# ahtamjidi/3PRE

Hardware: AMD Instinct MI355X
Metric: EKF steps/sec (predict+RANSAC+update) at N=500 landmarks; P-update %MFMA peak (higher is better)
Workload: dtype f32

## Files before the change

### 3pre_amd/csrc/pre3_api.hip

```cpp
#include <time.h>
#include <algorithm>
#include <immintrin.h>
#include <cmath>
#include <cstdarg>
#include <new>

#include <chrono>
#include "pre3_internal.h"
#include "pre3_test_hooks.h"
#include "pre3_geomdev.h"
#include <mutex>
#include "pre3_cholp.h"

namespace pre3 {

static thread_local char g_err[512] = "";
void set_error(const char *fmt, ...)
{
    va_list ap; va_start(ap, fmt);
    vsnprintf(g_err, sizeof g_err, fmt, ap);
    va_end(ap);
}

template <typename T> static int dmalloc(T **p, size_t count)
// ... 142 lines not shown
            if (t0 == 0) t0 = t;
            else if (t - t0 > 2.0) break;
        }
    }
    PRE3_TRY(stream_drain(c, __func__));
    if (__atomic_load_n(w, __ATOMIC_ACQUIRE) != seq) {
        c->stage_seq[k] = 0;
        (void)hipMemsetAsync(c->chol_arrive + 8 + k, 0, sizeof(unsigned int), c->stream);
        set_error("staging block %d: its pull has not run", k);
        return PRE3_E_STATE;
    }
    return PRE3_OK;
}
static StageDone stage_done(pre3_ctx *c, int k) { return StageDone{ c->chol_arrive + 8 + k, c->mail_dev + 16 + k, ++c->stage_seq[k] }; }

int launch_pull(pre3_ctx *c, const void *pinned_host, void *dst_dev, size_t bytes, int done_slot)
{
    void *src_dev = nullptr;
    PRE3_HIP(hipHostGetDevicePointer(&src_dev, const_cast<void *>(pinned_host), 0));
    const int n16 = (int)((bytes + 15) / 16);
    if (n16 == 0) return PRE3_OK;
    hipLaunchKernelGGL(k_scan_pull, dim3(ceil_div(n16, 256)), dim3(256), 0, c->stream, (const int4 *)src_dev, n16, (int4 *)dst_dev, 0, (int4 *)nullptr,
                       done_slot >= 0 ? stage_done(c, done_slot) : StageDone{ nullptr, nullptr, 0 });
    PRE3_HIP(hipGetLastError());
    return PRE3_OK;
}

int install_measurements(pre3_ctx *c, int m, const int32_t *meas_idx, const double *z, const int32_t *hyp, int n_hyp_ints, bool flags_clear, bool pull, size_t *nbytes_out)
{
    PRE3_CHECK(m >= 0 && m <= c->capm, PRE3_E_ARG, "measurements: m=%d exceeds capacity %d", m, c->capm);
    for (int j = 0; j < m; ++j) {
        PRE3_CHECK(meas_idx[j] >= 0 && meas_idx[j] < c->N, PRE3_E_ARG, "measurements: landmark index %d out of range", meas_idx[j]);
        PRE3_CHECK(j == 0 || meas_idx[j] > meas_idx[j - 1], PRE3_E_ARG, "measurements: landmark indices must be strictly ascending");
    }
    if (c->inbox_pending) { PRE3_TRY(wait_mail(c, 10, c->seq_inbox)); c->inbox_pending = false; }
    c->m = m; c->meas_host.assign(meas_idx, meas_idx + m);
    c->carry.select_pending = false;
    int32_t *hm = (int32_t *)(c->inbox_host + c->off_meas), *hic = (int32_t *)(c->inbox_host + c->off_ic);
    double *hz = (double *)(c->inbox_host + c->off_z);
    memset(hic, 0, sizeof(int32_t) * c->N);
    for (int j = 0; j < m; ++j) { hm[j] = meas_idx[j]; hic[meas_idx[j]] = 1; }
    if (z) {
        memset(hz, 0, sizeof(double) * 2 * c->N);
        for (int j = 0; j < m; ++j) { hz[2 * meas_idx[j]] = z[2 * j]; hz[2 * meas_idx[j] + 1] = z[2 * j + 1]; }
    }
    if (hyp) memcpy(c->inbox_host + c->off_hyp, hyp, sizeof(int32_t) * n_hyp_ints);
    const size_t nbytes = z ? c->off_z + sizeof(double) * 2 * c->N : c->off_hyp + (hyp ? sizeof(int32_t) * n_hyp_ints : 0);
    int32_t *const flags = (int32_t *)((unsigned char *)c->inbox_dev + c->off_flags);
    if (pull) { PRE3_TRY(launch_inbox_pull(c, c->inbox_host_dev, c->inbox_dev, (nbytes + 15) / 16, ++c->seq_inbox, 10, flags_clear ? nullptr : flags, flags_clear ? 0 : (int)(c->flags_bytes / 4))); c->inbox_pending = true; }
    if (nbytes_out) *nbytes_out = nbytes;
    if (!flags_clear && !pull) PRE3_HIP(hipMemsetAsync(flags, 0, c->flags_bytes, c->stream));
    c->li_from_host = c->hi_from_host = -1; c->li_kernel = c->hi_kernel = false;
    c->hp_all_valid = false;
    c->measurements_set = true;
    return PRE3_OK;
}

}

using namespace pre3;

extern "C" {

const char *pre3_last_error(void) { return pre3::g_err; }
const char *pre3_version(void) { return "pre3-mi355x 0.1 (gfx950)"; }

int pre3_device_count(void)
{
    int n = 0;
    if (hipGetDeviceCount(&n) != hipSuccess) return 0;
    return n;
}

static int pend_alloc(pre3_ctx *c)
{
    if (c->W_pend && c->Wp_pend && c->hf_xy) return PRE3_OK;
    PRE3_CHECK(c->dtype == PRE3_F32 && c->Wp != nullptr && c->rcap >= 2 * NB, PRE3_E_STATE, "PRE3_OPT_PEND_HI: fp32 contexts with the persistent factorisation only");
    int rc = PRE3_OK;
    auto A = [&](int r) { if (rc == PRE3_OK) rc = r; };
    if (!c->W_pend) { void *f = nullptr; A(dmalloc_bytes(&f, (size_t)2 * NB * c->ldw * sizeof(float))); c->W_pend = (float *)f; }
    if (!c->Wp_pend) A(dmalloc_bytes(&c->Wp_pend, (size_t)ceil_div(c->ldw, 128) * (c->rcap / 16) * (3 * 4 * 64) * 16));
    if (!c->hf_xy) { void *f = nullptr; A(dmalloc_bytes(&f, sizeof(unsigned) * 256)); c->hf_xy = (unsigned *)f; }
    return rc;
}

static int tail_alloc(pre3_ctx *c)
{
    if (c->tail_yp && c->tail_hb && c->tail_hib && c->tail_wt) return PRE3_OK;
    PRE3_CHECK(c->dtype == PRE3_F32 && c->Wp != nullptr, PRE3_E_STATE, "PRE3_OPT_STEP_TAIL: fp32 contexts with the persistent factorisation only");
    int rc = PRE3_OK;
    auto A = [&](int r) { if (rc == PRE3_OK) rc = r; };
    if (!c->tail_yp) A(dmalloc_bytes(&c->tail_yp, (size_t)(c->capN + 1) * 2 * 3 * c->rcap * 2));
    if (!c->tail_hb) { void *f = nullptr; A(dmalloc_bytes(&f, (size_t)c->capN * 2 * 16 * sizeof(float))); c->tail_hb = (float *)f; }
    if (!c->tail_hib) { void *f = nullptr; A(dmalloc_bytes(&f, sizeof(int32_t) * (64 + 64 * 16))); c->tail_hib = (int32_t *)f; }
    if (!c->tail_wt) { void *f = nullptr; A(dmalloc_bytes(&f, (size_t)c->ldw * c->rcap * sizeof(float))); c->tail_wt = (float *)f; }
    return rc;
}

int pre3_create(pre3_ctx **out, int device, int dtype, int max_landmarks, int max_hyp)
{
    PRE3_CHECK(out != nullptr, PRE3_E_ARG, "pre3_create: null output pointer");
    *out = nullptr;
    PRE3_CHECK(dtype == PRE3_F64 || dtype == PRE3_F32, PRE3_E_ARG, "pre3_create: dtype must be PRE3_F64 or PRE3_F32");
    PRE3_CHECK(max_landmarks >= 1 && max_hyp >= 1, PRE3_E_ARG, "pre3_create: capacities must be >= 1");
    int ndev = 0;
    if (hipGetDeviceCount(&ndev) != hipSuccess || ndev <= 0) { set_error("no HIP device available (libpre3 has no CPU fallback)"); return PRE3_E_NODEVICE; }
    PRE3_CHECK(device >= 0 && device < ndev, PRE3_E_NODEVICE, "pre3_create: device %d out of range (have %d)", device, ndev);
    PRE3_HIP(hipSetDevice(device));
    pre3_ctx *c = new (std::nothrow) pre3_ctx();
    PRE3_CHECK(c != nullptr, PRE3_E_NOMEM, "out of host memory");
    c->device = device; c->dtype = dtype; c->esz = dtype == PRE3_F64 ? 8 : 4;
    c->capN = max_landmarks; c->capn = 13 + 6 * max_landmarks; c->capm = max_landmarks; c->caph = max_hyp;
    c->ld = round_up(c->capn, TILE); c->ldw = c->ld + NB;
    { const char *e = getenv("PRE3_TAIL"); c->step_tail = e ? atoi(e) != 0 : false; }
    c->rcap = round_up(2 * c->capm, NB) + NB;
    c->mask_words_cap = ceil_div(c->capm, 32);
    int rc = PRE3_OK;
    auto A = [&](int r) { if (rc == PRE3_OK) rc = r; };
    if (hipStreamCreateWithFlags(&c->stream, hipStreamNonBlocking) != hipSuccess) { set_error("hipStreamCreate failed"); delete c; return PRE3_E_HIP; }
    A(dmalloc(&c->x_kk, c->capn)); A(dmalloc(&c->x_km1, c->capn));
    A(dmalloc_bytes(&c->P, (size_t)c->ld * c->ld * c->esz));
    A(dmalloc(&c->lm.type, c->capN)); A(dmalloc(&c->lm.off, c->capN));
    A(dmalloc(&c->lm.h, 2 * (size_t)c->capN)); A(dmalloc(&c->lm.has_h, c->capN));
    A(dmalloc(&c->lm.Hc, 14 * (size_t)c->capN)); A(dmalloc(&c->lm.Hl, 12 * (size_t)c->capN));
    A(dmalloc(&c->lm.S, 4 * (size_t)c->capN)); A(dmalloc(&c->lm.has_S, c->capN));
    {
        c->off_meas = 0;
        c->off_ic = c->off_meas + sizeof(int32_t) * c->capm;
        c->off_hyp = (c->off_ic + sizeof(int32_t) * c->capN + 15) / 16 * 16;
        c->off_z = (c->off_hyp + sizeof(int32_t) * (size_t)c->caph * MAXK + 15) / 16 * 16;
        c->off_flags = c->off_z + sizeof(double) * 2 * c->capN;
        const size_t off_li = c->off_flags, off_hi = off_li + sizeof(int32_t) * c->capN;
        const size_t off_lim = off_hi + sizeof(int32_t) * c->capN, off_him = off_lim + sizeof(int32_t) * c->capm;
        c->flags_bytes = sizeof(int32_t) * (2 * (size_t)c->capN + 2 * (size_t)c->capm);
        c->inbox_bytes = c->off_flags + c->flags_bytes;
        A(dmalloc_bytes(&c->inbox_dev, c->inbox_bytes));
        if (rc == PRE3_OK && hipHostMalloc((void **)&c->inbox_host, c->inbox_bytes, hipHostMallocMapped) != hipSuccess) { set_error("hipHostMalloc failed"); rc = PRE3_E_NOMEM; }
        if (rc == PRE3_OK && hipHostGetDevicePointer((void **)&c->inbox_host_dev, c->inbox_host, 0) != hipSuccess) { set_error("hipHostGetDevicePointer failed"); rc = PRE3_E_HIP; }
        if (rc == PRE3_OK) {
            memset(c->inbox_host, 0, c->inbox_bytes);
            unsigned char *d = (unsigned char *)c->inbox_dev;
            c->meas = (int32_t *)(d + c->off_meas); c->lm.ic = (int32_t *)(d + c->off_ic);
            c->lm.li = (int32_t *)(d + off_li); c->lm.hi = (int32_t *)(d + off_hi); c->li_meas = (int32_t *)(d + off_lim); c->hi_meas = (int32_t *)(d + off_him);
            c->hyp = (int32_t *)(d + c->off_hyp); c->lm.z = (double *)(d + c->off_z);
        }
    }
    A(dmalloc(&c->row_col, (size_t)c->rcap * ELLW)); A(dmalloc_bytes(&c->row_val, (size_t)c->rcap * ELLW * c->esz));
    A(dmalloc(&c->row_nu, c->rcap));
    A(dmalloc_bytes(&c->HP, (size_t)c->rcap * c->ldw * c->esz));
    A(dmalloc_bytes(&c->W, (size_t)c->rcap * c->ldw * c->esz));
    A(dmalloc_bytes(&c->G, (size_t)c->rcap * c->rcap * c->esz));
    A(dmalloc_bytes(&c->Smat, (size_t)c->rcap * c->rcap * c->esz));
    A(dmalloc(&c->sel_rows, c->rcap)); A(dmalloc(&c->need, c->capm));
    if (rc == PRE3_OK) (void)hipMemset(c->need, 0, sizeof(int32_t) * c->capm);
    A(dmalloc(&c->support, (size_t)c->caph + 4 + (size_t)c->caph * c->mask_words_cap));
    if (rc == PRE3_OK) c->masks = reinterpret_cast<uint32_t *>(c->support + c->caph + 4);
    A(dmalloc(&c->stats, 16));
    A(dmalloc(&c->pred_params, 128));
    {
        const int nt = c->ld / 64, ns = ceil_div(nt, 4);
        std::vector<std::vector<int2>> lists(8);
        int sidx = 0;
        for (int SI = 0; SI < ns; ++SI)
            for (int SJ = SI; SJ < ns; ++SJ) {
                int best = 0;
                for (int x = 1; x < 8; ++x) if (lists[x].size() < lists[best].size()) best = x;
                (void)sidx;
                for (int i = SI * 4; i < std::min(nt, SI * 4 + 4); ++i)
                    for (int j = SJ * 4; j < std::min(nt, SJ * 4 + 4); ++j)
                        if (j >= i) lists[best].push_back(make_int2(i, j));
            }
        for (;;) {
            int lo = 0, hi = 0;
            for (int x = 1; x < 8; ++x) { if (lists[x].size() < lists[lo].size()) lo = x; if (lists[x].size() > lists[hi].size()) hi = x; }
            if (lists[hi].size() <= lists[lo].size() + 1) break;
            lists[lo].push_back(lists[hi].back());
            lists[hi].pop_back();
        }
        size_t mx = 1;
        int cnts[8];
        for (int x = 0; x < 8; ++x) { mx = std::max(mx, lists[x].size()); cnts[x] = (int)lists[x].size(); }
        std::vector<int2> flat(mx * 8, make_int2(0, 0));
        int total = 0;
        for (int x = 0; x < 8; ++x) { for (size_t k2 = 0; k2 < lists[x].size(); ++k2) flat[x * mx + k2] = lists[x][k2]; total += cnts[x]; }
        c->tiles_stride = (int)mx;
        c->n_tiles = total;
        {
            std::vector<int2> inter;
            size_t pos[8] = { 0 };
            while ((int)inter.size() < total)
                for (int x = 0; x < 8 && (int)inter.size() < total; ++x)
                    if (pos[x] < lists[x].size()) inter.push_back(lists[x][pos[x]++]);
            A(dmalloc_bytes(&c->tiles_flat, sizeof(int2) * (inter.size() ? inter.size() : 1)));
            if (rc == PRE3_OK && hipMemcpy(c->tiles_flat, inter.data(), sizeof(int2) * inter.size(), hipMemcpyHostToDevice) != hipSuccess) { set_error("tile table upload failed"); rc = PRE3_E_HIP; }
        }
        A(dmalloc(&c->tile_ctr, 8)); A(dmalloc(&c->tile_cnt, 8)); A(dmalloc(&c->chol_arrive, 16));
        if (rc == PRE3_OK) (void)hipMemset(c->chol_arrive, 0, sizeof(unsigned int) * 16);
        if (rc == PRE3_OK) { (void)hipMemset(c->tile_ctr, 0, sizeof(unsigned int) * 8); (void)hipMemcpy(c->tile_cnt, cnts, sizeof(cnts), hipMemcpyHostToDevice); }
        { hipDeviceProp_t pr; if (hipGetDeviceProperties(&pr, device) == hipSuccess && pr.multiProcessorCount > 0) c->num_cus = pr.multiProcessorCount; }
        A(dmalloc_bytes(&c->tiles, sizeof(int2) * flat.size()));
        if (rc == PRE3_OK && hipMemcpy(c->tiles, flat.data(), sizeof(int2) * flat.size(), hipMemcpyHostToDevice) != hipSuccess) { set_error("tile table upload failed"); rc = PRE3_E_HIP; }
    }
    if (dtype == PRE3_F32) {
        { const char *e = getenv("PRE3_K9_B3"); c->k9_b3 = e ? atoi(e) != 0 : true; }
        A(dmalloc_bytes(&c->Wp, (size_t)(c->ld + 128) * c->rcap * 6));
        A(dmalloc_bytes(&c->Sp, (size_t)(c->rcap / NB) * (c->rcap / NB) * 1536 * 16));
        { void *f = nullptr; A(dmalloc_bytes(&f, cholp_flag_bytes(c->ldw / 32))); c->cholp_flags = (unsigned int *)f; }
        {
            std::vector<int32_t> rec; std::vector<int2> t64;
            dd_build_groups(c->ld / 64, rec, t64, c->dd_tile_off);
            c->dd_n_groups = (int)c->dd_tile_off.size() - 1;
            { void *f = nullptr; A(dmalloc_bytes(&f, sizeof(int32_t) * rec.size())); c->dd_groups = (int32_t *)f; }
            A(dmalloc_bytes(&c->dd_tiles, sizeof(int2) * t64.size()));
            if (rc == PRE3_OK && (hipMemcpy(c->dd_groups, rec.data(), sizeof(int32_t) * rec.size(), hipMemcpyHostToDevice) != hipSuccess ||
                                  hipMemcpy(c->dd_tiles, t64.data(), sizeof(int2) * t64.size(), hipMemcpyHostToDevice) != hipSuccess)) { set_error("consumer table upload failed"); rc = PRE3_E_HIP; }
        }
        A(dmalloc_bytes(&c->cholp_tp, (size_t)(c->rcap / NB) * 1536 * 16));
        { void *f = nullptr; A(dmalloc_bytes(&f, sizeof(float) * 4 * (size_t)c->ld)); c->jn_q = (float *)f; }
        { void *f = nullptr; A(dmalloc_bytes(&f, sizeof(unsigned long long) * (2 * NB) * (2 * NB))); c->hf_sx = (unsigned long long *)f; }
        if (c->step_tail) A(tail_alloc(c));
        { const char *e = getenv("PRE3_PEND_HI"); if (e && atoi(e) != 0 && c->rcap >= 2 * NB && c->rcap / NB <= CP_MAX_NRB + 1) { A(pend_alloc(c)); c->pend_opt = rc == PRE3_OK; } }
        if (rc == PRE3_OK) { cholp_context_count(c->device, +1); c->cholp_counted = true; }
        const int nt = c->ld / 128, ns = ceil_div(nt, 4);
        std::vector<std::vector<int2>> lists(8);
        for (int SI = 0; SI < ns; ++SI)
            for (int SJ = SI; SJ < ns; ++SJ) {
                int best = 0;
                for (int x = 1; x < 8; ++x) if (lists[x].size() < lists[best].size()) best = x;
                for (int i = SI * 4; i < std::min(nt, SI * 4 + 4); ++i)
                    for (int j = SJ * 4; j < std::min(nt, SJ * 4 + 4); ++j)
                        if (j >= i) lists[best].push_back(make_int2(i, j));
            }
        for (;;) {
            int lo = 0, hi = 0;
            for (int x = 1; x < 8; ++x) { if (lists[x].size() < lists[lo].size()) lo = x; if (lists[x].size() > lists[hi].size()) hi = x; }
            if (lists[hi].size() <= lists[lo].size() + 1) break;
            lists[lo].push_back(lists[hi].back());
            lists[hi].pop_back();
        }
        std::vector<int2> inter;
        const int total = nt * (nt + 1) / 2;
        size_t pos[8] = { 0 };
        while ((int)inter.size() < total)
            for (int x = 0; x < 8 && (int)inter.size() < total; ++x)
                if (pos[x] < lists[x].size()) inter.push_back(lists[x][pos[x]++]);
        const int n_big = total <= c->num_cus ? total : total / c->num_cus * c->num_cus;
        int n_small_src = total - n_big;
        std::vector<int2> big, small;
        for (int pass = 0; pass < 2; ++pass)
            for (int k2 = (int)inter.size() - 1; k2 >= 0 && n_small_src > 0; --k2) {
                int2 &t = inter[k2];
                if (t.x < 0 || (pass == 0 && t.x != t.y)) continue;
                for (int a2 = 0; a2 < 2; ++a2)
                    for (int b2 = 0; b2 < 2; ++b2)
                        if (t.x != t.y || b2 >= a2) small.push_back(make_int2(2 * t.x + a2, 2 * t.y + b2));
                t.x = -1; --n_small_src;
            }
        for (const int2 &t : inter) if (t.x >= 0) big.push_back(make_int2((2 * t.x) | (1 << 16), 2 * t.y));
        inter = big;
        inter.insert(inter.end(), small.begin(), small.end());
        c->n_tiles128 = (int)inter.size();
        A(dmalloc_bytes(&c->tiles128, sizeof(int2) * inter.size()));
        if (rc == PRE3_OK && hipMemcpy(c->tiles128, inter.data(), sizeof(int2) * inter.size(), hipMemcpyHostToDevice) != hipSuccess) { set_error("tile table upload failed"); rc = PRE3_E_HIP; }
    }
    if (rc == PRE3_OK && hipHostMalloc((void **)&c->pinned_stats, sizeof(int32_t) * 16) != hipSuccess) { set_error("hipHostMalloc failed"); rc = PRE3_E_NOMEM; }
    if (rc == PRE3_OK && hipHostMalloc((void **)&c->mail_host, sizeof(int32_t) * 32, hipHostMallocMapped) != hipSuccess) { set_error("hipHostMalloc failed"); rc = PRE3_E_NOMEM; }
    if (rc == PRE3_OK) {
        memset(c->mail_host, 0, sizeof(int32_t) * 32);
        if (hipHostGetDevicePointer((void **)&c->mail_dev, c->mail_host, 0) != hipSuccess) { set_error("hipHostGetDevicePointer failed"); rc = PRE3_E_HIP; }
    }
    if (rc == PRE3_OK && (hipEventCreate(&c->t0) != hipSuccess || hipEventCreate(&c->t1) != hipSuccess)) { set_error("hipEventCreate failed"); rc = PRE3_E_HIP; }
    if (rc != PRE3_OK) { pre3_destroy(c); return rc; }
    (void)hipMemsetAsync(c->stats, 0, sizeof(int32_t) * 16, c->stream);
    (void)hipMemsetAsync(c->P, 0, (size_t)c->ld * c->ld * c->esz, c->stream);
    (void)stream_drain(c, __func__);
    *out = c;
    return PRE3_OK;
}

int pre3_destroy(pre3_ctx *c)
{
    if (!c) return PRE3_OK;
    (void)hipSetDevice(c->device);
    if (c->stream) (void)stream_drain(c, __func__);
    if (c->comm && !comm_abort_wait(c->comm, comm_abort_ms(c->comm))) set_error("pre3_destroy: the communicator's abort has not returned: buffers are freed under it");
    else if (c->comm && comm_broken(c->comm) && c->stream) (void)stream_drain(c, __func__);
    if (c->cholp_counted) { cholp_context_count(c->device, -1); c->cholp_counted = false; }
    ic_rank_free(c);
    if (c->comm && c->comm_owned) (void)pre3_comm_destroy((pre3_comm *)c->comm);
    c->comm = nullptr;
    void *bufs[] = { c->x_kk, c->x_km1, c->P, c->lm.type, c->lm.off, c->lm.h, c->lm.has_h, c->lm.Hc, c->lm.Hl, c->lm.S, c->lm.has_S,
                     c->inbox_dev, c->row_col, c->row_val, c->row_nu, c->HP, c->W, c->G, c->Smat, c->Rdense,
                     c->sel_rows, c->support, c->stats, c->pred_params, c->tiles, c->tile_ctr, c->tile_cnt, c->tiles_flat, c->P_alt, c->x_alt, c->map_col, c->map_val, c->map_desc, c->map_src0, c->map_conv, c->map_feat, c->map_flags, c->bank, c->bank_alt, c->scan_desc, c->scan_pos, c->ic_pred, c->ic_counts, c->ic_arg, c->ic_newk2, c->ic_best, c->ic_second, c->bank_src, c->chol_arrive, c->ic_pb, c->ic_ps, c->ic_pa, c->Wp, c->Sp, c->tiles128, c->need, c->cholp_flags, c->cholp_tp, c->dd_groups, c->dd_tiles, c->tail_yp, c->tail_hb, c->tail_hib, c->tail_wt, c->jn_q, c->W_pend, c->Wp_pend, c->hf_xy, c->hf_sx };
    for (void *b : bufs) if (b) (void)hipFree(b);
    free_readers(c);
    free_rows(c);
    free_plane(c);
    free_policy(c);
    for (int k2 = 0; k2 < 2; ++k2) { if (c->map_stage[k2]) (void)hipHostFree(c->map_stage[k2]); if (c->map_stage_ev[k2]) (void)hipEventDestroy(c->map_stage_ev[k2]); }
    for (int k2 = 0; k2 < 2; ++k2) { if (c->up_stage[k2]) (void)hipHostFree(c->up_stage[k2]); if (c->up_stage_ev[k2]) (void)hipEventDestroy(c->up_stage_ev[k2]); }
    if (c->pinned_stats) (void)hipHostFree(c->pinned_stats);
    if (c->inbox_host) (void)hipHostFree(c->inbox_host);
    if (c->mail_host) (void)hipHostFree(c->mail_host);
    if (c->ic_result_host) (void)hipHostFree(c->ic_result_host);
    for (hipEvent_t e : c->kt.ev) (void)hipEventDestroy(e);
    if (c->t0) (void)hipEventDestroy(c->t0);
    if (c->t1) (void)hipEventDestroy(c->t1);
    if (c->stream) (void)hipStreamDestroy(c->stream);
    delete c;
    return PRE3_OK;
}

int pre3_set_option(pre3_ctx *c, int option, int value)
{
    EntryScope scope(c); PRE3_TRY(scope.rc);
    switch (option) {
    case PRE3_OPT_DEFER_HI: c->defer_hi = value != 0; return PRE3_OK;
    case PRE3_OPT_K9_BF16X3: c->k9_b3 = value != 0 && c->dtype == PRE3_F32 && c->Wp != nullptr; return PRE3_OK;
    case PRE3_OPT_CHOL_PERSIST: c->chol_persist = value != 0; return PRE3_OK;
    case PRE3_OPT_K9_OVERLAP: c->k9_overlap = value != 0; return PRE3_OK;
    case PRE3_OPT_STEP_TAIL:
        if (value != 0 && c->dtype == PRE3_F32 && c->Wp != nullptr) { const int rc = tail_alloc(c); if (rc != PRE3_OK) { c->step_tail = false; return rc; } }
        c->step_tail = value != 0;
        return PRE3_OK;
    case PRE3_OPT_PEND_HI:
        if (value != 0 && c->dtype == PRE3_F32 && c->Wp != nullptr && c->rcap / NB <= CP_MAX_NRB + 1) { const int rc = pend_alloc(c); if (rc != PRE3_OK) { c->pend_opt = false; return rc; } }
        c->pend_opt = value != 0 && c->W_pend != nullptr;
        return PRE3_OK;
    default: set_error("pre3_set_option: unknown option %d", option); return PRE3_E_ARG;
    }
}

int pre3_get_option(pre3_ctx *c, int option, int *value_out)
{
    PRE3_CHECK(c != nullptr && value_out != nullptr, PRE3_E_ARG, "pre3_get_option: null argument");
    switch (option) {
    case PRE3_OPT_DEFER_HI: *value_out = c->defer_hi ? 1 : 0; return PRE3_OK;
    case PRE3_OPT_K9_BF16X3: *value_out = c->k9_b3 ? 1 : 0; return PRE3_OK;
    case PRE3_OPT_CHOL_PERSIST: *value_out = cholp_usable(c, 1) ? 1 : 0; return PRE3_OK;
    case PRE3_OPT_IC_RANKED: *value_out = c->ic_last_ranked ? 1 : 0; return PRE3_OK;
    case PRE3_OPT_IC_ROUTE: *value_out = c->ic_route; return PRE3_OK;
    case PRE3_OPT_K9_OVERLAP: *value_out = c->k9_overlap ? 1 : 0; return PRE3_OK;
    case PRE3_OPT_STEP_TAIL: *value_out = (c->step_tail && c->tail_yp != nullptr) ? 1 : 0; return PRE3_OK;
    case PRE3_OPT_PEND_HI: *value_out = c->pend_opt ? 1 : 0; return PRE3_OK;
    case PRE3_OPT_ROWS_FORM: *value_out = c->rows_form; return PRE3_OK;
    default: set_error("pre3_get_option: unknown option %d", option); return PRE3_E_ARG;
    }
}

int pre3_sync(pre3_ctx *c)
{
    EntryScope scope(c); PRE3_TRY(scope.rc);
    PRE3_TRY(stream_drain(c, __func__));
    return PRE3_OK;
}

int pre3_set_cam(pre3_ctx *c, const pre3_cam *cam)
{
    EntryScope scope(c); PRE3_TRY(scope.rc);
    PRE3_CHECK(cam != nullptr && cam->f > 0, PRE3_E_ARG, "pre3_set_cam: invalid camera");
    c->cam = *cam; c->have_cam = true;
    return PRE3_OK;
}

int pre3_set_map(pre3_ctx *c, int N, const int32_t *lm_type)
{
    EntryScope scope(c); PRE3_TRY(scope.rc);
    PRE3_CHECK(N >= 0 && N <= c->capN, PRE3_E_ARG, "pre3_set_map: N=%d exceeds capacity %d", N, c->capN);
    PRE3_CHECK(N == 0 || lm_type != nullptr, PRE3_E_ARG, "pre3_set_map: null type list");
    std::vector<int32_t> off(N ? N : 1);
    int n = 13;
    for (int i = 0; i < N; ++i) {
        PRE3_CHECK(lm_type[i] == PRE3_INVDEPTH || lm_type[i] == PRE3_CARTESIAN, PRE3_E_ARG, "pre3_set_map: landmark %d has unknown type %d", i, lm_type[i]);
        off[i] = n; n += lm_type[i] == PRE3_INVDEPTH ? 6 : 3;
    }
    PRE3_CHECK(n <= c->capn, PRE3_E_ARG, "pre3_set_map: state size %d exceeds capacity %d", n, c->capn);
    PRE3_TRY(stream_drain(c, __func__));
    if (N) {
        PRE3_HIP(hipMemcpy(c->lm.type, lm_type, sizeof(int32_t) * N, hipMemcpyHostToDevice));
        PRE3_HIP(hipMemcpy(c->lm.off, off.data(), sizeof(int32_t) * N, hipMemcpyHostToDevice));
    }
    c->N = N; c->n = n;
    c->lm_type_host.assign(lm_type, lm_type + N);
    PRE3_HIP(hipMemset(c->lm.has_h, 0, sizeof(int32_t) * c->capN)); PRE3_HIP(hipMemset(c->lm.has_S, 0, sizeof(int32_t) * c->capN));
    PRE3_HIP(hipMemset(c->lm.h, 0, sizeof(double) * 2 * c->capN)); PRE3_HIP(hipMemset(c->lm.Hc, 0, sizeof(double) * 14 * c->capN));
    PRE3_HIP(hipMemset(c->lm.Hl, 0, sizeof(double) * 12 * c->capN)); PRE3_HIP(hipMemset(c->lm.S, 0, sizeof(double) * 4 * c->capN));
    PRE3_HIP(hipMemset(c->inbox_dev, 0, c->inbox_bytes)); PRE3_HIP(hipMemset(c->lm.li, 0, sizeof(int32_t) * c->capN));
    PRE3_HIP(hipMemset(c->lm.hi, 0, sizeof(int32_t) * c->capN));
    c->m = 0; c->meas_host.clear(); c->measurements_set = false; c->projected = false; c->innovated = false;
    c->x_valid[0] = c->x_valid[1] = false; c->p_which = -1;
    c->booked = false; c->book_s = 0;
    return PRE3_OK;
}

int pre3_state_size(pre3_ctx *c) { return c ? c->n : PRE3_E_ARG; }

int pre3_set_state(pre3_ctx *c, int which, int n, const double *x, const double *P)
{
    EntryScope scope(c);
    if (c == nullptr || (scope.rc != PRE3_OK && scope.rc != PRE3_E_NUMERIC && scope.rc != PRE3_E_HIP)) return scope.rc;
    PRE3_HIP(hipSetDevice(c->device));
    (void)stream_drain(c, __func__);
    (void)hipMemsetAsync(c->stats + 6, 0, sizeof(int32_t) * 2, c->stream);
    if (c->mail_host) { c->mail_host[6] = 0; c->mail_host[7] = 0; }
    drop_carried(c);
    PRE3_CHECK(which == PRE3_X_K_K || which == PRE3_X_K_KM1, PRE3_E_ARG, "pre3_set_state: bad selector");
    PRE3_CHECK(n == c->n, PRE3_E_ARG, "pre3_set_state: n=%d but the map defines n=%d", n, c->n);
    PRE3_CHECK(x && P, PRE3_E_ARG, "pre3_set_state: null pointer");
    PRE3_TRY(stream_drain(c, __func__));
    PRE3_HIP(hipMemcpy(which == PRE3_X_K_K ? c->x_kk : c->x_km1, x, sizeof(double) * n, hipMemcpyHostToDevice));
    const int ld = c->ld;
    PRE3_HIP(hipMemset(c->P, 0, (size_t)ld * ld * c->esz));
    if (c->dtype == PRE3_F64) {
        PRE3_HIP(hipMemcpy2D(c->P, (size_t)ld * 8, P, (size_t)n * 8, (size_t)n * 8, n, hipMemcpyHostToDevice));
    } else {
        std::vector<float> tmp((size_t)n * n);
        for (size_t i = 0; i < (size_t)n * n; ++i) tmp[i] = (float)P[i];
        PRE3_HIP(hipMemcpy2D(c->P, (size_t)ld * 4, tmp.data(), (size_t)n * 4, (size_t)n * 4, n, hipMemcpyHostToDevice));
    }
    c->x_valid[which] = true; c->p_which = which; c->hp_all_valid = false;
    return PRE3_OK;
}

int pre3_get_state(pre3_ctx *c, int which, int n, double *x, double *P)
{
    EntryScope scope(c); PRE3_TRY(scope.rc);
    PRE3_CHECK(which == PRE3_X_K_K || which == PRE3_X_K_KM1, PRE3_E_ARG, "pre3_get_state: bad selector");
    PRE3_CHECK(n == c->n, PRE3_E_ARG, "pre3_get_state: n=%d but the map defines n=%d", n, c->n);
    PRE3_CHECK(c->x_valid[which], PRE3_E_STATE, "pre3_get_state: that estimate has not been computed");
    PRE3_TRY(fetch_stats(c));
    if (x) PRE3_HIP(hipMemcpy(x, which == PRE3_X_K_K ? c->x_kk : c->x_km1, sizeof(double) * n, hipMemcpyDeviceToHost));
    if (P) {
        PRE3_CHECK(c->p_which == which, PRE3_E_STATE, "pre3_get_state: the covariance buffer currently holds the other estimate (it is updated in place)");
        const int ld = c->ld;
        if (c->dtype == PRE3_F64) {
            PRE3_HIP(hipMemcpy2D(P, (size_t)n * 8, c->P, (size_t)ld * 8, (size_t)n * 8, n, hipMemcpyDeviceToHost));
        } else {
            std::vector<float> tmp((size_t)n * n);
            PRE3_HIP(hipMemcpy2D(tmp.data(), (size_t)n * 4, c->P, (size_t)ld * 4, (size_t)n * 4, n, hipMemcpyDeviceToHost));
            for (size_t i = 0; i < (size_t)n * n; ++i) P[i] = (double)tmp[i];
        }
    }
    return PRE3_OK;
}

static int reader_precheck(pre3_ctx *c, int which, const char *who)
// ... 728 lines not shown
```

### 3pre_amd/csrc/pre3_geom.hip

```cpp
#include "pre3_internal.h"
#include "pre3_geomdev.h"
#include "pre3_chain.h"

namespace pre3 {

__device__ inline void d_process_noise(double *Pn)
{
    for (int i = 0; i < 49; ++i) Pn[i] = 0;
    double sx = 0.01 / 3; sx = sx * sx;
    Pn[0] = Pn[8] = Pn[16] = sx;
    const double PI = 3.141592653589793238462643383279502884;
    double a = 0.24 / 2 * PI / 180;
    double e[3] = { a * 1, a * 0.1, a * 1 };
    double sr = sin(e[0] / 2), sp = sin(e[1] / 2), sy = sin(e[2] / 2);
    double cr = cos(e[0] / 2), cp = cos(e[1] / 2), cy = cos(e[2] / 2);
    double Qe[12] = {
        0.5 * (-cy * cp * sr + sy * sp * cr), 0.5 * (-cy * sp * cr + sy * cp * sr), 0.5 * (-sy * cp * cr + cy * sp * sr),
        0.5 * ( cy * cp * cr + sy * sp * sr), 0.5 * (-cy * sp * sr - sy * cp * cr), 0.5 * (-sy * cp * sr - cy * sp * cr),
        0.5 * (-cy * sp * sr + sy * cp * cr), 0.5 * ( cy * cp * cr - sy * sp * sr), 0.5 * (-sy * sp * cr + cy * cp * sr),
        0.5 * (-sy * cp * sr - cy * sp * cr), 0.5 * (-cy * cp * sr - sy * sp * cr), 0.5 * ( cy * cp * cr + sy * sp * sr) };
    for (int i = 0; i < 4; ++i)
        for (int j = 0; j < 4; ++j) {
            double s = 0;
            for (int t = 0; t < 3; ++t) s += (Qe[i * 3 + t] * (e[t] * e[t])) * Qe[j * 3 + t];
// ... 186 lines not shown
    int j = blockIdx.x * blockDim.x + threadIdx.x;
    bool strip = j < n && (j < 3 || j >= 7);
    double v[4] = { 0, 0, 0, 0 };
    if (strip) for (int t = 0; t < 4; ++t) v[t] = (double)P[(3 + t) * ld + j];
    __syncthreads();
    if (strip) {
        for (int i = 0; i < 4; ++i) {
            const double b = jn_row(sJn, i, v);
            P[(3 + i) * ld + j] = (T)b; P[j * ld + 3 + i] = (T)b;
        }
    }
    if (blockIdx.x == 0 && threadIdx.x == 0) {
        double T1[16];
        for (int i = 0; i < 4; ++i) for (int k = 0; k < 4; ++k) { const double w[4] = { corner[k], corner[4 + k], corner[8 + k], corner[12 + k] }; T1[i * 4 + k] = jn_row(sJn, i, w); }
        for (int i = 0; i < 4; ++i) for (int k = 0; k < 4; ++k) P[(3 + i) * ld + 3 + k] = (T)jn_row(sJn, k, &T1[i * 4]);
    }
}

__global__ void k_project(int N, const int32_t *__restrict__ lm_type, const int32_t *__restrict__ lm_off,
                          const double *__restrict__ x, CamD cam, int clear_first,
                          double *__restrict__ h, int32_t *__restrict__ has_h, double *__restrict__ Hc, double *__restrict__ Hl)
{
    int i = blockIdx.x * blockDim.x + threadIdx.x;
    if (i >= N) return;
    project_one(i, lm_type, lm_off, x, cam, clear_first, h, has_h, Hc, Hl);
}


struct HiArgs { int fuse, m, seq; const int32_t *meas; int32_t *hi_meas, *sel_rows, *stats, *mail; unsigned int *done; };
__device__ __forceinline__ void collect_hi_body(int m, const int32_t *__restrict__ meas, const int32_t *__restrict__ lm_ic,
                                                const int32_t *__restrict__ lm_li, const int32_t *lm_hi,
                                                int32_t *__restrict__ hi_meas, int32_t *__restrict__ sel_rows, int32_t *__restrict__ stats,
                                                int32_t *mail, int seq);

__device__ __forceinline__ void hi_tail(const HiArgs &ha, const int32_t *__restrict__ ic, const int32_t *__restrict__ li, int32_t *hi)
{
    if (!ha.fuse) return;
    __shared__ int s_last;
    __syncthreads();
    if (threadIdx.x == 0) {
        __threadfence();
        s_last = atomicAdd(ha.done, 1u) == gridDim.x - 1;
    }
    __syncthreads();
    if (s_last && threadIdx.x < 64) {
        __builtin_amdgcn_fence(__ATOMIC_ACQUIRE, "agent");
        if (threadIdx.x == 0) *ha.done = 0;
        collect_hi_body(ha.m, ha.meas, ic, li, hi, ha.hi_meas, ha.sel_rows, ha.stats, ha.mail, ha.seq);
    }
}

template <typename T>
__global__ __launch_bounds__(256) void k_innovation(int N, const int32_t *__restrict__ lm_type, const int32_t *__restrict__ lm_off,
                                                    const T *__restrict__ P, int ld, const double *__restrict__ Hc, const double *__restrict__ Hl,
                                                    const int32_t *__restrict__ has_h, int mode, double chi2,
                                                    const double *__restrict__ h, const double *__restrict__ z,
                                                    const int32_t *__restrict__ ic, const int32_t *__restrict__ li, int32_t *__restrict__ hi,
                                                    double *__restrict__ S, int32_t *__restrict__ has_S, int32_t *__restrict__ clear, int n_clear,
                                                    HiArgs ha)
{
    for (int t = blockIdx.x * blockDim.x + threadIdx.x; t < n_clear; t += gridDim.x * blockDim.x) clear[t] = 0;
    innovation_body<T>(N, lm_type, lm_off, P, ld, Hc, Hl, has_h, mode, chi2, h, z, ic, li, hi, S, has_S, blockIdx.x * blockDim.x + threadIdx.x);
    hi_tail(ha, ic, li, hi);
}

template <typename T>
__global__ __launch_bounds__(256) void k_project_innovation(int N, const int32_t *__restrict__ lm_type, const int32_t *__restrict__ lm_off,
                                                            const double *__restrict__ x, CamD cam, int clear_first, const T *__restrict__ P, int ld,
                                                            double *Hc, double *Hl, int32_t *has_h, int mode, double chi2, double *h,
                                                            const double *__restrict__ z, const int32_t *__restrict__ ic,
                                                            const int32_t *__restrict__ li, int32_t *__restrict__ hi, double *__restrict__ S,
                                                            int32_t *__restrict__ has_S, int32_t *__restrict__ clear, int n_clear, HiArgs ha,
                                                            int32_t *__restrict__ clear2, int n_clear2, IcMatchRide mr)
{
    const int n_main = gridDim.x - mr.n_blocks;
    if (mr.n_blocks > 0) {
        __shared__ double Qs[ICS_T][ICS_LD], Bs[ICS_T][ICS_LD];
        if ((int)blockIdx.x >= n_main) { ic_match_tile(mr, blockIdx.x - n_main, Qs, Bs); return; }
    }
    const int gt = blockIdx.x * blockDim.x + threadIdx.x;
    for (int t = gt; t < n_clear; t += n_main * blockDim.x) clear[t] = 0;
    for (int t = gt; t < n_clear2; t += n_main * blockDim.x) clear2[t] = 0;
    if (threadIdx.x < 16 && (int)(blockIdx.x * 16 + threadIdx.x) < N) project_one(blockIdx.x * 16 + threadIdx.x, lm_type, lm_off, x, cam, clear_first, h, has_h, Hc, Hl);
    __threadfence_block();
    __syncthreads();
    innovation_body<T>(N, lm_type, lm_off, P, ld, Hc, Hl, has_h, mode, chi2, h, z, ic, li, hi, S, has_S, blockIdx.x * blockDim.x + threadIdx.x);
    hi_tail(ha, ic, li, hi);
}

__global__ void k_window_gate(int M, const int32_t *__restrict__ pred_idx, const int32_t *__restrict__ k1,
                              const double *__restrict__ zc, const double *__restrict__ h, const double *__restrict__ S,
                              const int32_t *__restrict__ has_S, int strict, double *__restrict__ z, int32_t *__restrict__ ic,
                              int32_t *__restrict__ accept)
{
    int c = blockIdx.x * blockDim.x + threadIdx.x;
    if (c >= M) return;
    int lm = pred_idx[k1[c]];
    int slm = strict ? pred_idx[c] : lm;
    double half = has_S[slm] ? ceil(3 * sqrt(S[4 * slm])) : 40.0;
    double dx = zc[2 * c] - h[2 * lm], dy = zc[2 * c + 1] - h[2 * lm + 1];
    int ok = sqrt(dx * dx + dy * dy) <= half;
    if (ok) { ic[lm] = 1; z[2 * lm] = zc[2 * c]; z[2 * lm + 1] = zc[2 * c + 1]; }
    if (accept) accept[c] = ok;
}

template <typename T>
__global__ void k_build_rows(int nsel, const int32_t *__restrict__ sel, const int32_t *__restrict__ meas,
                             const int32_t *__restrict__ lm_type, const int32_t *__restrict__ lm_off,
                             const double *__restrict__ Hc, const double *__restrict__ Hl,
                             const double *__restrict__ z, const double *__restrict__ h,
                             int32_t *__restrict__ row_col, T *__restrict__ row_val, double *__restrict__ row_nu, int r_pad)
{
    int a = blockIdx.x * blockDim.x + threadIdx.x;
    if (a >= r_pad) return;
    int32_t *cc = row_col + a * ELLW;
    T *vv = row_val + a * ELLW;
    if (a >= 2 * nsel) {
        for (int t = 0; t < ELLW; ++t) { cc[t] = 0; vv[t] = (T)0; }
        row_nu[a] = 0;
        return;
    }
    int s = a >> 1, c = a & 1;
    int i = meas[sel ? sel[s] : s];
    int d = lm_type[i] == PRE3_INVDEPTH ? 6 : 3;
    int off = lm_off[i];
    for (int t = 0; t < 7; ++t) { cc[t] = t; vv[t] = (T)Hc[14 * i + c * 7 + t]; }
    for (int t = 0; t < 6; ++t) { cc[7 + t] = t < d ? off + t : 0; vv[7 + t] = t < d ? (T)Hl[12 * i + c * 6 + t] : (T)0; }
    for (int t = 13; t < ELLW; ++t) { cc[t] = 0; vv[t] = (T)0; }
    row_nu[a] = z[2 * i + c] - h[2 * i + c];
}

__device__ inline double wave_min(double v)
{
    for (int o = 32; o > 0; o >>= 1) v = fmin(v, __shfl_xor(v, o, 64));
    return v;
}
__device__ inline int wave_sum(int v)
{
    for (int o = 32; o > 0; o >>= 1) v += __shfl_xor(v, o, 64);
    return v;
}

struct SelArgs {
    int fuse, n_draw, k, early_exit, seq;
    int32_t *li_meas, *lm_li, *sel_rows, *stats, *mail;
    unsigned int *done;
};
__device__ __forceinline__ void select_body(int n_draw, int k, int early_exit, int m, const int32_t *__restrict__ meas,
                                            int32_t *support, const uint32_t *masks, int mask_words,
                                            int32_t *__restrict__ li_meas, int32_t *__restrict__ lm_li,
                                            int32_t *__restrict__ sel_rows, int32_t *__restrict__ stats,
                                            int32_t *mail, int seq, int err_idx = -1);

template <typename T, int K>
__global__ __launch_bounds__(512) void k_ransac_score(int hyp_begin, const int32_t *__restrict__ hyp, int m,
                                                      const int32_t *__restrict__ meas, const int32_t *__restrict__ lm_type,
                                                      const int32_t *__restrict__ lm_off, const double *__restrict__ x,
                                                      const T *__restrict__ HP, int ldw, const T *__restrict__ G, int ldg,
                                                      const double *__restrict__ row_nu, const double *__restrict__ z,
                                                      CamD cam, double threshold, int32_t *support,
                                                      uint32_t *masks, int mask_words, SelArgs sel,
                                                      const int32_t *__restrict__ row_col, const T *__restrict__ row_val)
{
    constexpr int R = 2 * K;
    extern __shared__ double s_res[];
    __shared__ double s_w[R];
    __shared__ double s_red[8];
    __shared__ int s_cnt[8];
    const int hidx = hyp_begin + blockIdx.x;
    const int tid = threadIdx.x, lane = tid & 63, wv = tid >> 6;
    int rows[R];
#pragma unroll
    for (int s = 0; s < K; ++s) { const int j = hyp[hidx * K + s]; rows[2 * s] = 2 * j; rows[2 * s + 1] = 2 * j + 1; }
    const T *hp[R];
#pragma unroll
    for (int b = 0; b < R; ++b) hp[b] = HP + (size_t)rows[b] * ldw;
    constexpr bool PRE_POSE = R * sizeof(T) <= 48;
    T hpc[R][7];
    double xp[7];
#pragma unroll
    for (int c = 0; c < 7; ++c) {
        xp[c] = x[c];
        if (PRE_POSE) {
#pragma unroll
            for (int b = 0; b < R; ++b) hpc[b][c] = hp[b][c];
        }
    }
    const bool have0 = PRE_POSE && tid < m;
    int i0 = 0, type0 = PRE3_INVDEPTH;
    T hpl[R][6];
    double xl[6], z0 = 0, z1 = 0;
    if (have0) {
        i0 = meas[tid];
        type0 = lm_type[i0];
        const int off = lm_off[i0];
        struct __attribute__((packed, aligned(sizeof(T)))) Row6 { T v[6]; };
        struct __attribute__((packed, aligned(8))) X6 { double v[6]; };
        const X6 xv = *reinterpret_cast<const X6 *>(x + off);
#pragma unroll
        for (int b = 0; b < R; ++b) {
            const Row6 rv = *reinterpret_cast<const Row6 *>(hp[b] + off);
#pragma unroll
            for (int c = 0; c < 6; ++c) hpl[b][c] = (c < 3 || type0 == PRE3_INVDEPTH) ? rv.v[c] : (T)0;
        }
#pragma unroll
        for (int c = 0; c < 6; ++c) xl[c] = (c < 3 || type0 == PRE3_INVDEPTH) ? xv.v[c] : 0.0;
        z0 = z[2 * i0]; z1 = z[2 * i0 + 1];
    }
    const int solver = (int)(blockDim.x >> 6) - 1;
    if (wv == solver) {
        double A[R][R + 1];
        T gv = (T)0;
        if (G == nullptr) {
            int pi = 0;
            while ((pi + 1) * (pi + 2) / 2 <= lane) ++pi;
            const int pj = lane - pi * (pi + 1) / 2;
            if (pi < R) {
                int ri = 0, rj = 0;
#pragma unroll
                for (int a = 0; a < R; ++a) { if (a == pi) ri = rows[a]; if (a == pj) rj = rows[a]; }
                const int ra = ri > rj ? ri : rj, rb = ri > rj ? rj : ri;
                T vv[ELLW]; int cc[ELLW];
#pragma unroll
                for (int t = 0; t < ELLW; ++t) { vv[t] = row_val[rb * ELLW + t]; cc[t] = row_col[rb * ELLW + t]; }
                T hv[ELLW];
#pragma unroll
                for (int t = 0; t < ELLW; ++t) hv[t] = HP[(size_t)ra * ldw + cc[t]];
#pragma unroll
                for (int t = 0; t < ELLW; ++t) gv = ell_fma(vv[t], hv[t], gv);
            }
        }
#pragma unroll
        for (int a = 0; a < R; ++a) {
#pragma unroll
            for (int b = 0; b < R; ++b) {
                if (G != nullptr) {
                    const int ra = rows[a] > rows[b] ? rows[a] : rows[b], rb = rows[a] > rows[b] ? rows[b] : rows[a];
                    A[a][b] = (double)G[(size_t)ra * ldg + rb] + (a == b ? 1.0 : 0.0);
                } else {
                    const int hi_ = a > b ? a : b, lo_ = a > b ? b : a;
                    A[a][b] = (double)__shfl(gv, hi_ * (hi_ + 1) / 2 + lo_, 64) + (a == b ? 1.0 : 0.0);
                }
            }
            A[a][R] = row_nu[rows[a]];
        }
        if (lane == 0) {
#pragma unroll
            for (int c = 0; c < R; ++c) {
                int p = c; double best = fabs(A[c][c]);
#pragma unroll
                for (int a = c + 1; a < R; ++a) { double v = fabs(A[a][c]); if (v > best) { best = v; p = a; } }
#pragma unroll
                for (int a = c + 1; a < R; ++a)
                    if (a == p) {
#pragma unroll
                        for (int b = 0; b <= R; ++b) { double t = A[c][b]; A[c][b] = A[a][b]; A[a][b] = t; }
                    }
                const double dinv = 1.0 / A[c][c];
#pragma unroll
                for (int a = c + 1; a < R; ++a) {
                    const double l = A[a][c] * dinv;
#pragma unroll
                    for (int b = c + 1; b <= R; ++b) A[a][b] -= l * A[c][b];
                }
            }
            double w[R];
#pragma unroll
            for (int a = R - 1; a >= 0; --a) {
                double s = A[a][R];
#pragma unroll
                for (int b = a + 1; b < R; ++b) s -= A[a][b] * w[b];
                w[a] = s / A[a][a];
            }
#pragma unroll
            for (int a = 0; a < R; ++a) s_w[a] = w[a];
        }
    }
    __syncthreads();
    double w[R];
#pragma unroll
    for (int b = 0; b < R; ++b) w[b] = s_w[b];
    double xc[7];
#pragma unroll
    for (int c = 0; c < 7; ++c) {
        double s = 0;
#pragma unroll
        for (int b = 0; b < R; ++b) s += w[b] * (double)(PRE_POSE ? hpc[b][c] : hp[b][c]);
        xc[c] = xp[c] + s;
    }
    double rot[9];
    d_q2r(xc + 3, rot);
    double lmin = INFINITY;
    for (int j = tid; j < m; j += blockDim.x) {
        const bool pre = PRE_POSE && j == tid;
        const int i = pre ? i0 : meas[j];
        const int type = pre ? type0 : lm_type[i], off = pre ? 0 : lm_off[i];
        double y[6];
#pragma unroll
        for (int c = 0; c < 6; ++c) {
            double s = 0;
            if (c < 3 || type == PRE3_INVDEPTH) {
#pragma unroll
                for (int b = 0; b < R; ++b) s += w[b] * (double)(pre ? hpl[b][c] : hp[b][off + c]);
                s += pre ? xl[c] : x[off + c];
            }
            y[c] = s;
        }
        double v[3], hc[3];
        d_ray(type, y, xc, v);
#pragma unroll
        for (int c = 0; c < 3; ++c) hc[c] = rot[0 * 3 + c] * v[0] + rot[1 * 3 + c] * v[1] + rot[2 * 3 + c] * v[2];
        double uvd[2];
        d_pinhole_distort(hc, cam, uvd);
        const double n0 = (pre ? z0 : z[2 * i]) - uvd[0], n1 = (pre ? z1 : z[2 * i + 1]) - uvd[1];
        const double res = sqrt(n0 * n0 + n1 * n1);
        s_res[j] = res;
        if (type == PRE3_INVDEPTH) lmin = fmin(lmin, res);
    }
    lmin = wave_min(lmin);
    if (lane == 0) s_red[wv] = lmin;
    uint32_t *s_mask = (uint32_t *)(s_res + m);
    for (int wd = tid; wd < mask_words; wd += blockDim.x) s_mask[wd] = 0;
    __syncthreads();
    double minres = s_red[0];
    for (int w2 = 1; w2 < (int)(blockDim.x >> 6); ++w2) minres = fmin(minres, s_red[w2]);
    int cnt = 0;
    for (int j = tid; j < m; j += blockDim.x) {
        const int type = lm_type[meas[j]];
        const double res = s_res[j];
        const int in = (type == PRE3_INVDEPTH) ? (res < (minres + threshold)) : (res < threshold);
        if (in) { atomicOr(&s_mask[j >> 5], 1u << (j & 31)); ++cnt; }
    }
    cnt = wave_sum(cnt);
    if (lane == 0) s_cnt[wv] = cnt;
    __syncthreads();
    if (tid == 0) { int sc = 0; for (int w2 = 0; w2 < (int)(blockDim.x >> 6); ++w2) sc += s_cnt[w2]; support[hidx] = sc; }
    for (int wd = tid; wd < mask_words; wd += blockDim.x) masks[(size_t)hidx * mask_words + wd] = s_mask[wd];
    if (sel.fuse) {
        __shared__ int s_last;
        __syncthreads();
        if (tid == 0) {
            __threadfence();
            s_last = atomicAdd(sel.done, 1u) == gridDim.x - 1;
        }
        __syncthreads();
        if (s_last) {
            __builtin_amdgcn_fence(__ATOMIC_ACQUIRE, "agent");
            if (tid == 0) *sel.done = 0;
            select_body(sel.n_draw, sel.k, sel.early_exit, m, meas, support, masks, mask_words, sel.li_meas, sel.lm_li, sel.sel_rows,
                        sel.stats, sel.mail, sel.seq);
        }
    }
}

__device__ inline int wave_compact(int flag, int lane, int base_cnt, int32_t *__restrict__ dst, int value)
{
    unsigned long long mask = __ballot(flag);
    int pos = __popcll(mask & ((1ull << lane) - 1ull));
    if (flag) dst[base_cnt + pos] = value;
    return base_cnt + __popcll(mask);
}

__device__ inline int ransac_n_hyp(int sup, int m)
{
    double epsilon = 1 - ((double)sup / (double)m);
    return (int)ceil(log(1 - 0.99) / log(1 - (1 - epsilon)));
}

struct SelBest { int best, iters, n_hyp, max_support; };
__device__ __forceinline__ SelBest select_find_best(int n_draw, int k, int early_exit, int m, const int32_t *support)
{
    __shared__ int s_stop[4];
    __shared__ unsigned long long s_key[4];
    const int tid = threadIdx.x, lane = tid & 63, wv = tid >> 6;
    const bool act = tid < 256;
    const int limit = early_exit ? (n_draw < 1000 ? n_draw : 1000) : n_draw;
    int v4[4];
#pragma unroll
    for (int q = 0; q < 4; ++q) { const int it = tid + 256 * q; v4[q] = (act && it < limit) ? support[it] : -1; }
    int e = limit;
    if (early_exit) {
        int mine = 0x7fffffff;
#pragma unroll
        for (int q = 3; q >= 0; --q) if (v4[q] >= 1 && ransac_n_hyp(v4[q], m) <= k) mine = tid + 256 * q;
        for (int o = 32; o > 0; o >>= 1) mine = min(mine, __shfl_xor(mine, o, 64));
        if (act && lane == 0) s_stop[wv] = mine;
        __syncthreads();
        const int first = min(min(s_stop[0], s_stop[1]), min(s_stop[2], s_stop[3]));
        if (first < limit) e = first;
    }
    unsigned long long key = 0;
#pragma unroll
    for (int q = 0; q < 4; ++q) {
        const int it = tid + 256 * q;
        if (it <= e && v4[q] >= 1) key = max(key, ((unsigned long long)v4[q] << 32) | (unsigned long long)(0xffffffffu - (unsigned)it));
    }
    for (int it = tid + 1024; act && it < limit; it += 256) {
        const int v = support[it];
        if (v >= 1) key = max(key, ((unsigned long long)v << 32) | (unsigned long long)(0xffffffffu - (unsigned)it));
    }
    for (int o = 32; o > 0; o >>= 1) key = max(key, (unsigned long long)__shfl_xor((long long)key, o, 64));
    if (act && lane == 0) s_key[wv] = key;
    __syncthreads();
    key = max(max(s_key[0], s_key[1]), max(s_key[2], s_key[3]));
    SelBest r;
    r.best = key ? (int)(0xffffffffu - (unsigned)(key & 0xffffffffull)) : -1;
    r.max_support = (int)(key >> 32);
    r.iters = e < limit ? e + 1 : limit;
    r.n_hyp = r.best >= 0 ? ransac_n_hyp(r.max_support, m) : 1000;
    return r;
}

__device__ __forceinline__ void select_body(int n_draw, int k, int early_exit, int m, const int32_t *__restrict__ meas,
                                            int32_t *support, const uint32_t *masks, int mask_words,
                                            int32_t *__restrict__ li_meas, int32_t *__restrict__ lm_li,
                                            int32_t *__restrict__ sel_rows, int32_t *__restrict__ stats,
                                            int32_t *mail, int seq, int err_idx)
{
    __shared__ int s_wcnt[4], s_base;
    const int tid = threadIdx.x, lane = tid & 63, wv = tid >> 6;
    if (tid == 0) s_base = 0;
    const SelBest sb = select_find_best(n_draw, k, early_exit, m, support);
    if (tid == 0) { stats[0] = sb.best; stats[1] = sb.iters; stats[2] = sb.n_hyp; stats[3] = sb.max_support; }
    const int best = sb.best, iters = sb.iters;
    const bool act = tid < 256;
    for (int it = iters + tid; act && it < n_draw; it += 256) support[it] = -1;
    for (int base = 0; base < m; base += 256) {
        const int j = base + tid;
        int in = 0;
        if (act && j < m) {
            in = best >= 0 ? (masks[(size_t)best * mask_words + (j >> 5)] >> (j & 31)) & 1 : 0;
            li_meas[j] = in; lm_li[meas[j]] = in;
        }
        const unsigned long long bal = __ballot(in);
        if (act && lane == 0) s_wcnt[wv] = __popcll(bal);
        __syncthreads();
        int pre = s_base;
        for (int w2 = 0; w2 < wv && w2 < 4; ++w2) pre += s_wcnt[w2];
        if (in) sel_rows[pre + __popcll(bal & ((1ull << lane) - 1ull))] = j;
        else if (act && j < m) sel_rows[m + j - (pre + __popcll(bal & ((1ull << lane) - 1ull)))] = (j << 16) | (meas[j] & 0xffff);
        __syncthreads();
        if (tid == 0) s_base += s_wcnt[0] + s_wcnt[1] + s_wcnt[2] + s_wcnt[3];
        __syncthreads();
    }
    if (tid == 0) {
        stats[4] = s_base;
        mail[0] = sb.best; mail[1] = sb.iters; mail[2] = sb.n_hyp; mail[3] = sb.max_support; mail[4] = s_base;
        mail[11] = err_idx >= 0 ? support[err_idx] : 0;
        __threadfence_system();
        __hip_atomic_store(&mail[8], seq, __ATOMIC_RELEASE, __HIP_MEMORY_SCOPE_SYSTEM);
    }
}

__global__ __launch_bounds__(256) void k_ransac_select(int n_draw, int k, int early_exit, int m, const int32_t *__restrict__ meas,
                                                       int32_t *__restrict__ support, const uint32_t *__restrict__ masks, int mask_words,
                                                       int32_t *__restrict__ li_meas, int32_t *__restrict__ lm_li,
                                                       int32_t *__restrict__ sel_rows, int32_t *__restrict__ stats,
                                                       int32_t *mail, int seq, int err_idx)
{
    select_body(n_draw, k, early_exit, m, meas, support, masks, mask_words, li_meas, lm_li, sel_rows, stats, mail, seq, err_idx);
}

constexpr int SG_RB = 8;
constexpr int SG_MAXW = 64;
constexpr int SGL_RB = 4;

__device__ __forceinline__ int select_local_list(int n_draw, int k, int early_exit, int m, const int32_t *support, const uint32_t *masks, int mask_words,
                                                 int *s_sel )
{
    __shared__ int s_pre[SG_MAXW + 1];
    __shared__ uint32_t s_word[SG_MAXW];
    const int tid = threadIdx.x, lane = tid & 63, wv = tid >> 6;
    const int best = select_find_best(n_draw, k, early_exit, m, support).best;
    if (wv == 0) {
        uint32_t wd = (best >= 0 && lane < mask_words) ? masks[(size_t)best * mask_words + lane] : 0u;
        if (lane == mask_words - 1 && (m & 31)) wd &= (1u << (m & 31)) - 1u;
        int inc = __popc(wd);
#pragma unroll
        for (int o = 1; o < 64; o <<= 1) { int t = __shfl_up(inc, o, 64); if (lane >= o) inc += t; }
        s_word[lane] = wd; s_pre[lane + 1] = inc;
        if (lane == 0) s_pre[0] = 0;
    }
    __syncthreads();
    for (int j = tid; j < m; j += 256) {
        const uint32_t wd = s_word[j >> 5];
        if ((wd >> (j & 31)) & 1u) s_sel[s_pre[j >> 5] + __popc(wd & ((1u << (j & 31)) - 1u))] = j;
    }
    __syncthreads();
    return s_pre[mask_words];
}
// ... 219 lines not shown
    }
    if (blockIdx.x == 0) {
        if (rg == 0 && i >= 3 && i < 7) q[i - 3] = s;
        __syncthreads();
        if (rg == 0 && i == 0) { double Jn[16]; d_normjac(q, Jn); for (int t = 0; t < 16; ++t) { params[16 + t] = Jn[t]; params[96 + t] = Jn[t]; } }
        if (rg == 0 && i >= 3 && i < 7) s = s / sqrt(q[0] * q[0] + q[1] * q[1] + q[2] * q[2] + q[3] * q[3]);
    }
    if (rg == 0 && i < n) x_out[i] = s;
}

static CamD to_camd(const pre3_cam &c) { return CamD{ c.f, c.Cx, c.Cy, c.k1, c.k2, c.nRows, c.nCols }; }

#define DISPATCH_T(c, expr_f64, expr_f32) do { if ((c)->dtype == PRE3_F64) { expr_f64; } else { expr_f32; } } while (0)

ProjRide make_proj_ride(pre3_ctx *c, int which, int clear_first, int slot, int n_producers)
{
    ProjRide pr{};
    pr.n_blocks = ceil_div(c->N, 64); pr.N = c->N; pr.clear_first = clear_first;
    pr.lm_type = c->lm.type; pr.lm_off = c->lm.off; pr.x = which == PRE3_X_K_K ? c->x_kk : c->x_km1; pr.cam = to_camd(c->cam);
    pr.h = c->lm.h; pr.has_h = c->lm.has_h; pr.Hc = c->lm.Hc; pr.Hl = c->lm.Hl;
    pr.ctr = c->chol_arrive + 3 + slot;
    pr.guard = c->stats + 7;
    c->ride_target[slot] += (unsigned)n_producers;
    pr.target = c->ride_target[slot];
    return pr;
}

int launch_predict_impl(pre3_ctx *c, const double u[7], bool with_projection, size_t inbox_n16, int32_t inbox_seq)
{
    U7 uu; for (int i = 0; i < 7; ++i) uu.v[i] = u[i];
    int blocks = ceil_div(c->n, 256);
    ProjRide pr{};
    static const int own_pose = getenv("PRE3_RIDE_POSE") ? atoi(getenv("PRE3_RIDE_POSE")) : 1;
    if (with_projection && c->N > 0) {
        pr = make_proj_ride(c, PRE3_X_K_KM1, 1, 0, own_pose ? 0 : 1); pr.x_lm = c->x_kk;
        pr.own_pose = own_pose ? 1 : 0; pr.x_prev = c->x_kk; pr.u = uu;
    }
    InboxRide ib{ (const int4 *)c->inbox_host_dev, (int4 *)c->inbox_dev, (int)inbox_n16, c->mail_dev, inbox_seq };
    const int nb = blocks + pr.n_blocks + (inbox_n16 ? 1 : 0);
    const int fuse_jn = c->carry.jn_pending ? 1 : 0;
    DISPATCH_T(c,
        hipLaunchKernelGGL(k_predict<double>, dim3(nb), dim3(256), 0, c->stream, c->x_kk, c->x_km1, (double *)c->P, c->n, c->ld, uu, c->pred_params, blocks, pr, ib, fuse_jn, PendW{}),
        hipLaunchKernelGGL(k_predict<float>, dim3(nb), dim3(256), 0, c->stream, c->x_kk, c->x_km1, (float *)c->P, c->n, c->ld, uu, c->pred_params, blocks, pr, ib, fuse_jn, pend_args(c)));
    PRE3_HIP(hipGetLastError());
    c->carry.jn_pending = false;
    return PRE3_OK;
}

int launch_jnorm(pre3_ctx *c, int)
{
    PRE3_TRY(pend_flush(c));
    int blocks = ceil_div(c->n, 256);
    ProjRide pr{};
    GateRide<float> gr{};
    static const int gate_env = getenv("PRE3_GATE_RIDE") ? atoi(getenv("PRE3_GATE_RIDE")) : 1;
    if (c->out.proj_with_jnorm && c->N > 0) {
        if (gate_env && c->req.want_gate_ride && c->out.jn_q_valid && c->dtype == PRE3_F32) {
            gr.n_blocks = ceil_div(c->N, 16); gr.N = c->N; gr.Q = c->jn_q; gr.chi2 = c->req.rescue_chi2; gr.project = c->out.proj_in_cholp ? 0 : 1;
            gr.lm_type = c->lm.type; gr.lm_off = c->lm.off; gr.x = c->x_kk; gr.cam = to_camd(c->cam);
            gr.h = c->lm.h; gr.has_h = c->lm.has_h; gr.Hc = c->lm.Hc; gr.Hl = c->lm.Hl; gr.z = c->lm.z; gr.ic = c->lm.ic; gr.li = c->lm.li; gr.hi = c->lm.hi;
            c->out.rescue_gated = true;
        } else {
            pr = make_proj_ride(c, PRE3_X_K_K, 0, 1, 0);
        }
        c->out.rescue_projected = true;
    }
    c->out.proj_with_jnorm = false; c->out.proj_in_cholp = false;
    c->out.jn_q_valid = false;
    DISPATCH_T(c,
        hipLaunchKernelGGL(k_jnorm_P<double>, dim3(blocks + pr.n_blocks), dim3(256), 0, c->stream, (double *)c->P, c->n, c->ld, c->pred_params, blocks, pr, GateRide<double>{}),
        hipLaunchKernelGGL(k_jnorm_P<float>, dim3(blocks + pr.n_blocks + gr.n_blocks), dim3(256), 0, c->stream, (float *)c->P, c->n, c->ld, c->pred_params, blocks, pr, gr));
    PRE3_HIP(hipGetLastError());
    return PRE3_OK;
}

int launch_project(pre3_ctx *c, int which, int clear_first)
{
    const double *x = which == PRE3_X_K_K ? c->x_kk : c->x_km1;
    hipLaunchKernelGGL(k_project, dim3(ceil_div(c->N, 64)), dim3(64), 0, c->stream, c->N, c->lm.type, c->lm.off, x, to_camd(c->cam),
                       clear_first, c->lm.h, c->lm.has_h, c->lm.Hc, c->lm.Hl);
    PRE3_HIP(hipGetLastError());
    return PRE3_OK;
}


int launch_project_innovation(pre3_ctx *c, int which, int clear_first, int mode, double chi2, bool collect, bool clear_ic, const IcMatchRide *ride)
{
    PRE3_TRY(pend_flush(c));
    const IcMatchRide mr = ride ? *ride : IcMatchRide{};
    const double *x = which == PRE3_X_K_K ? c->x_kk : c->x_km1;
    int32_t *clr = (int32_t *)((unsigned char *)c->inbox_dev + c->off_flags);
    const int n_clr = mode == 0 ? (int)(c->flags_bytes / sizeof(int32_t)) : 0;
    HiArgs ha{};
    if (mode == 1 && collect) ha = HiArgs{ hi_fuse() ? 1 : 0, c->m, ++c->seq_collect, c->meas, c->hi_meas, c->sel_rows, c->stats, c->mail_dev, c->chol_arrive + 2 };
    dim3 g(ceil_div(c->N * 16, 256) + mr.n_blocks), b(256);
    DISPATCH_T(c,
        hipLaunchKernelGGL(k_project_innovation<double>, g, b, 0, c->stream, c->N, c->lm.type, c->lm.off, x, to_camd(c->cam), clear_first,
                           (const double *)c->P, c->ld, c->lm.Hc, c->lm.Hl, c->lm.has_h, mode, chi2, c->lm.h, c->lm.z, c->lm.ic, c->lm.li,
                           c->lm.hi, c->lm.S, c->lm.has_S, clr, n_clr, ha, clear_ic ? c->lm.ic : nullptr, clear_ic ? c->N : 0, mr),
        hipLaunchKernelGGL(k_project_innovation<float>, g, b, 0, c->stream, c->N, c->lm.type, c->lm.off, x, to_camd(c->cam), clear_first,
                           (const float *)c->P, c->ld, c->lm.Hc, c->lm.Hl, c->lm.has_h, mode, chi2, c->lm.h, c->lm.z, c->lm.ic, c->lm.li,
                           c->lm.hi, c->lm.S, c->lm.has_S, clr, n_clr, ha, clear_ic ? c->lm.ic : nullptr, clear_ic ? c->N : 0, mr));
    PRE3_HIP(hipGetLastError());
    if (mode == 1 && collect && !ha.fuse) PRE3_TRY(launch_collect_hi(c, ha));
    return PRE3_OK;
}

int launch_innovation(pre3_ctx *c, int mode, double chi2, bool clear_flags, bool collect)
{
    PRE3_TRY(pend_flush(c));
    int32_t *clr = (int32_t *)((unsigned char *)c->inbox_dev + c->off_flags);
    const int n_clr = clear_flags ? (int)(c->flags_bytes / sizeof(int32_t)) : 0;
    HiArgs ha{};
    if (mode == 1 && collect) ha = HiArgs{ hi_fuse() ? 1 : 0, c->m, ++c->seq_collect, c->meas, c->hi_meas, c->sel_rows, c->stats, c->mail_dev, c->chol_arrive + 2 };
    dim3 g(ceil_div(c->N * 16, 256)), b(256);
    DISPATCH_T(c,
        hipLaunchKernelGGL(k_innovation<double>, g, b, 0, c->stream, c->N, c->lm.type, c->lm.off, (const double *)c->P, c->ld, c->lm.Hc,
                           c->lm.Hl, c->lm.has_h, mode, chi2, c->lm.h, c->lm.z, c->lm.ic, c->lm.li, c->lm.hi, c->lm.S, c->lm.has_S, clr, n_clr, ha),
        hipLaunchKernelGGL(k_innovation<float>, g, b, 0, c->stream, c->N, c->lm.type, c->lm.off, (const float *)c->P, c->ld, c->lm.Hc,
                           c->lm.Hl, c->lm.has_h, mode, chi2, c->lm.h, c->lm.z, c->lm.ic, c->lm.li, c->lm.hi, c->lm.S, c->lm.has_S, clr, n_clr, ha));
    PRE3_HIP(hipGetLastError());
    if (mode == 1 && collect && !ha.fuse) PRE3_TRY(launch_collect_hi(c, ha));
    return PRE3_OK;
}

int launch_window_gate(pre3_ctx *c, int M, const int32_t *pred_idx_dev, const int32_t *k1_dev, const double *zc_dev, int strict,
                       int32_t *accept_dev)
{
    hipLaunchKernelGGL(k_window_gate, dim3(ceil_div(M, 64)), dim3(64), 0, c->stream, M, pred_idx_dev, k1_dev, zc_dev, c->lm.h, c->lm.S,
                       c->lm.has_S, strict, c->lm.z, c->lm.ic, accept_dev);
    PRE3_HIP(hipGetLastError());
    return PRE3_OK;
}

int launch_build_rows_impl(pre3_ctx *c, int nsel, const int32_t *sel_dev, int r_pad)
{
    dim3 g(ceil_div(r_pad, 64)), b(64);
    DISPATCH_T(c,
        hipLaunchKernelGGL(k_build_rows<double>, g, b, 0, c->stream, nsel, sel_dev, c->meas, c->lm.type, c->lm.off, c->lm.Hc, c->lm.Hl,
                           c->lm.z, c->lm.h, c->row_col, (double *)c->row_val, c->row_nu, r_pad),
        hipLaunchKernelGGL(k_build_rows<float>, g, b, 0, c->stream, nsel, sel_dev, c->meas, c->lm.type, c->lm.off, c->lm.Hc, c->lm.Hl,
                           c->lm.z, c->lm.h, c->row_col, (float *)c->row_val, c->row_nu, r_pad));
    PRE3_HIP(hipGetLastError());
    return PRE3_OK;
}

constexpr int SCORE_THREADS = 512;

template <typename T>
static void launch_score_k(pre3_ctx *c, int k, int nb, size_t shm, int hyp_begin, double threshold, int ldg, int32_t *support_dev,
                           uint32_t *mask_dev, int mask_words, const SelArgs &sel)
{
#define SCORE_ARGS hyp_begin, c->hyp, c->m, c->meas, c->lm.type, c->lm.off, c->x_km1, (const T *)c->HP, c->ldw, c->g_valid ? (const T *)c->G : (const T *)nullptr, ldg, \
                   c->row_nu, c->lm.z, to_camd(c->cam), threshold, support_dev, mask_dev, mask_words, sel, c->row_col, (const T *)c->row_val
    switch (k) {
    case 1: hipLaunchKernelGGL((k_ransac_score<T, 1>), dim3(nb), dim3(SCORE_THREADS), shm, c->stream, SCORE_ARGS); break;
    case 2: hipLaunchKernelGGL((k_ransac_score<T, 2>), dim3(nb), dim3(SCORE_THREADS), shm, c->stream, SCORE_ARGS); break;
    case 3: hipLaunchKernelGGL((k_ransac_score<T, 3>), dim3(nb), dim3(SCORE_THREADS), shm, c->stream, SCORE_ARGS); break;
    default: hipLaunchKernelGGL((k_ransac_score<T, 4>), dim3(nb), dim3(SCORE_THREADS), shm, c->stream, SCORE_ARGS); break;
    }
#undef SCORE_ARGS
}

int launch_ransac_score_impl(pre3_ctx *c, int k, double threshold, int hyp_begin, int hyp_end, int ldg, int32_t *support_dev,
                             uint32_t *mask_dev, int mask_words, int select_n_draw, int early_exit)
{
    int nb = hyp_end - hyp_begin;
    if (nb <= 0) return PRE3_OK;
    size_t shm = sizeof(double) * c->m + sizeof(uint32_t) * mask_words + 16;
    SelArgs sel{};
    if (select_n_draw > 0) {
        sel = SelArgs{ 1, select_n_draw, k, early_exit, ++c->seq_select, c->li_meas, c->lm.li, c->sel_rows, c->stats, c->mail_dev, c->chol_arrive + 1 };
    }
    DISPATCH_T(c,
        launch_score_k<double>(c, k, nb, shm, hyp_begin, threshold, ldg, support_dev, mask_dev, mask_words, sel),
        launch_score_k<float>(c, k, nb, shm, hyp_begin, threshold, ldg, support_dev, mask_dev, mask_words, sel));
    PRE3_HIP(hipGetLastError());
    return PRE3_OK;
}

int launch_ransac_select_impl(pre3_ctx *c, int n_draw, int k, int early_exit, int32_t *support_dev, const uint32_t *mask_dev, int mask_words, int err_idx)
{
    hipLaunchKernelGGL(k_ransac_select, dim3(1), dim3(256), 0, c->stream, n_draw, k, early_exit, c->m, c->meas, support_dev, mask_dev,
                       mask_words, c->li_meas, c->lm.li, c->sel_rows, c->stats, c->mail_dev, ++c->seq_select, err_idx);
    PRE3_HIP(hipGetLastError());
    return PRE3_OK;
}

bool select_gather_usable(const pre3_ctx *c)
{
    static const int env = getenv("PRE3_SELECT_GATHER") ? atoi(getenv("PRE3_SELECT_GATHER")) : 1;
    return env && c->m > 0 && ceil_div(c->m, 32) <= SG_MAXW;
}

int launch_select_gather(pre3_ctx *c, int n_draw, int k, int early_exit, int mask_words)
{
    const int r_pad_max = round_up(2 * c->m, NB);
    const int seq = ++c->seq_select;
    static const int lds_env = getenv("PRE3_SELECT_GATHER_LDS") ? atoi(getenv("PRE3_SELECT_GATHER_LDS")) : 1;
    const size_t stage = (size_t)SGL_RB * c->ldw * (c->dtype == PRE3_F64 ? 8 : 4);
    const size_t stage1 = stage / SGL_RB;
    if (lds_env && stage > 55 * 1024 && stage1 <= 55 * 1024 && c->dtype == PRE3_F32) {
        const int ny = r_pad_max;
        dim3 g(ny + 1), b(256);
        hipLaunchKernelGGL((k_select_gather_lds<float, 1, 12>), g, b, stage1, c->stream, n_draw, k, early_exit, c->m, c->meas, c->support, c->masks, mask_words, c->li_meas, c->lm.li,
                           c->sel_rows, c->stats, c->mail_dev, seq, ny, (const float *)c->HP, (float *)c->W, c->ldw, c->row_col, (const float *)c->row_val, (float *)c->Smat);
        PRE3_HIP(hipGetLastError());
        return PRE3_OK;
    }
    if (lds_env && stage <= 55 * 1024) {
        const int ny = r_pad_max / SGL_RB;
        dim3 g(ny + 1), b(256);
        DISPATCH_T(c,
            hipLaunchKernelGGL((k_select_gather_lds<double, SGL_RB, 4>), g, b, stage, c->stream, n_draw, k, early_exit, c->m, c->meas, c->support, c->masks, mask_words, c->li_meas, c->lm.li,
                               c->sel_rows, c->stats, c->mail_dev, seq, ny, (const double *)c->HP, (double *)c->W, c->ldw, c->row_col, (const double *)c->row_val, (double *)c->Smat),
            hipLaunchKernelGGL((k_select_gather_lds<float, SGL_RB, 4>), g, b, stage, c->stream, n_draw, k, early_exit, c->m, c->meas, c->support, c->masks, mask_words, c->li_meas, c->lm.li,
                               c->sel_rows, c->stats, c->mail_dev, seq, ny, (const float *)c->HP, (float *)c->W, c->ldw, c->row_col, (const float *)c->row_val, (float *)c->Smat));
        PRE3_HIP(hipGetLastError());
        return PRE3_OK;
    }
    const int ny = r_pad_max / SG_RB;
    const int gxW = ceil_div(c->ldw / 4, 256);
    dim3 g(gxW + ceil_div(r_pad_max, 256), ny + 1), b(256);
    DISPATCH_T(c,
        hipLaunchKernelGGL(k_select_gather<double>, g, b, 0, c->stream, n_draw, k, early_exit, c->m, c->meas, c->support, c->masks, mask_words, c->li_meas, c->lm.li,
                           c->sel_rows, c->stats, c->mail_dev, seq, ny, gxW, (const double *)c->HP, (double *)c->W, c->ldw, c->row_col,
                           (const double *)c->row_val, (double *)c->Smat),
        hipLaunchKernelGGL(k_select_gather<float>, g, b, 0, c->stream, n_draw, k, early_exit, c->m, c->meas, c->support, c->masks, mask_words, c->li_meas, c->lm.li,
                           c->sel_rows, c->stats, c->mail_dev, seq, ny, gxW, (const float *)c->HP, (float *)c->W, c->ldw, c->row_col,
                           (const float *)c->row_val, (float *)c->Smat));
    PRE3_HIP(hipGetLastError());
    return PRE3_OK;
}

int launch_update_x(pre3_ctx *c, int which_prior, int r)
{
    const double *xp = which_prior == PRE3_X_K_K ? c->x_kk : c->x_km1;
    dim3 g(ceil_div(c->n, 64)), b(1024);
    DISPATCH_T(c,
        hipLaunchKernelGGL(k_update_x<double>, g, b, 0, c->stream, c->n, r, (const double *)c->W, c->ldw, c->ld, xp, c->x_kk, c->pred_params, c->tile_ctr),
        hipLaunchKernelGGL(k_update_x<float>, g, b, 0, c->stream, c->n, r, (const float *)c->W, c->ldw, c->ld, xp, c->x_kk, c->pred_params, c->tile_ctr));
    c->tile_ctr_clean = true;
    PRE3_HIP(hipGetLastError());
    return PRE3_OK;
}


__global__ __launch_bounds__(1024) void k_inbox_pull(InboxRide ib) { inbox_pull_block(ib); }

__global__ __launch_bounds__(1024) void k_slice_prepare(InboxRide ib, int32_t *__restrict__ zero, int n_zero, const int32_t *hyp, int k, int lo, int hi,
                                                        int32_t *__restrict__ need, int tag)
{
    if (blockIdx.x > 0) {
        int4 *z4 = reinterpret_cast<int4 *>(zero);
        for (int i = (blockIdx.x - 1) * 1024 + threadIdx.x; i < n_zero / 4; i += (gridDim.x - 1) * 1024) z4[i] = int4{ 0, 0, 0, 0 };
        if (blockIdx.x == 1 && (int)threadIdx.x < (n_zero & 3)) zero[(n_zero & ~3) + threadIdx.x] = 0;
        return;
    }
    if (ib.n16 > 0) inbox_pull_block(ib);
    else __syncthreads();
    for (int t = threadIdx.x; t < (hi - lo) * k; t += 1024) need[hyp[lo * k + t]] = tag;
}
int launch_slice_prepare(pre3_ctx *c, const void *src_host_mapped, size_t n16, int32_t seq, int n_zero, int k, int lo, int hi, int tag)
{
    hipLaunchKernelGGL(k_slice_prepare, dim3(1 + (n_zero > 0 ? std::min(16, ceil_div(n_zero, 4096)) : 0)), dim3(1024), 0, c->stream, InboxRide{ (const int4 *)src_host_mapped, (int4 *)c->hyp, (int)n16, c->mail_dev, seq, 10 },
                       c->support, n_zero, c->hyp, k, lo, hi, c->need, tag);
    PRE3_HIP(hipGetLastError());
    return PRE3_OK;
}
int launch_inbox_pull(pre3_ctx *c, const void *src_host_mapped, void *dst_dev, size_t n16, int32_t seq, int slot, int32_t *clear, int n_clear)
{
    hipLaunchKernelGGL(k_inbox_pull, dim3(1), dim3(1024), 0, c->stream, InboxRide{ (const int4 *)src_host_mapped, (int4 *)dst_dev, (int)n16, c->mail_dev, seq, slot, clear, n_clear });
    PRE3_HIP(hipGetLastError());
    return PRE3_OK;
}

__global__ __launch_bounds__(256) void k_hyp_support(const double *__restrict__ xi, CamD cam, int n_id, const int32_t *__restrict__ i1,
                                                     const int32_t *__restrict__ i2, const int32_t *__restrict__ i3, const double *__restrict__ z_id,
                                                     int n_euc, const int32_t *__restrict__ i4, const double *__restrict__ z_euc, double threshold,
                                                     double *__restrict__ res, int32_t *__restrict__ out )
{
    __shared__ double s_red[4];
    __shared__ int s_cnt[4];
    const int tid = threadIdx.x, lane = tid & 63, wv = tid >> 6;
    double rot[9];
    d_q2r(xi + 3, rot);
    double lmin = INFINITY;
    for (int j = tid; j < n_id + n_euc; j += 256) {
        const bool id = j < n_id;
        const int e = j - n_id;
        double y[6];
        if (id) { y[0] = xi[i1[3 * j]]; y[1] = xi[i1[3 * j + 1]]; y[2] = xi[i1[3 * j + 2]]; y[3] = xi[i2[2 * j]]; y[4] = xi[i2[2 * j + 1]]; y[5] = xi[i3[j]]; }
        else { y[0] = xi[i4[3 * e]]; y[1] = xi[i4[3 * e + 1]]; y[2] = xi[i4[3 * e + 2]]; y[3] = y[4] = y[5] = 0; }
        double v[3], hc[3], uvd[2];
        d_ray(id ? PRE3_INVDEPTH : PRE3_CARTESIAN, y, xi, v);
#pragma unroll
        for (int c = 0; c < 3; ++c) hc[c] = rot[0 * 3 + c] * v[0] + rot[1 * 3 + c] * v[1] + rot[2 * 3 + c] * v[2];
        d_pinhole_distort(hc, cam, uvd);
        const double *z = id ? z_id + 2 * j : z_euc + 2 * e;
        const double n0 = z[0] - uvd[0], n1 = z[1] - uvd[1];
        const double r = sqrt(n0 * n0 + n1 * n1);
        res[j] = r;
        if (id) lmin = fmin(lmin, r);
    }
    lmin = wave_min(lmin);
    if (lane == 0) s_red[wv] = lmin;
    __syncthreads();
    const double minres = fmin(fmin(s_red[0], s_red[1]), fmin(s_red[2], s_red[3]));
    int cnt = 0;
    for (int j = tid; j < n_id + n_euc; j += 256) {
        const int in = j < n_id ? (res[j] < (minres + threshold)) : (res[j] < threshold);
        out[1 + j] = in; cnt += in;
    }
    cnt = wave_sum(cnt);
    if (lane == 0) s_cnt[wv] = cnt;
    __syncthreads();
    if (tid == 0) out[0] = s_cnt[0] + s_cnt[1] + s_cnt[2] + s_cnt[3];
}

int run_hypothesis_support(int n, const double *xi, const pre3_cam &cam, int n_id, const int32_t *i1, const int32_t *i2, const int32_t *i3,
                           const double *z_id, int n_euc, const int32_t *i4, const double *z_euc, double threshold, int32_t *out_host)
{
    const int m = n_id + n_euc;
    const size_t nd = (size_t)n + 3 * (size_t)m, ni = 6 * (size_t)n_id + 3 * (size_t)n_euc + 1 + m;
    void *blk = nullptr; int slot = -1;
    PRE3_TRY(scratch_acquire(sizeof(double) * nd + sizeof(int32_t) * ni, &blk, &slot));
    struct Rel { int slot; void *p; ~Rel() { scratch_release(slot, p); } } rel{ slot, blk };
    std::vector<double> hd(nd, 0.0);
    std::vector<int32_t> hi(ni, 0);
    memcpy(hd.data(), xi, sizeof(double) * n);
    if (n_id) memcpy(hd.data() + n, z_id, sizeof(double) * 2 * n_id);
    if (n_euc) memcpy(hd.data() + n + 2 * (size_t)n_id, z_euc, sizeof(double) * 2 * n_euc);
    if (n_id) { memcpy(hi.data(), i1, sizeof(int32_t) * 3 * n_id); memcpy(hi.data() + 3 * (size_t)n_id, i2, sizeof(int32_t) * 2 * n_id); memcpy(hi.data() + 5 * (size_t)n_id, i3, sizeof(int32_t) * n_id); }
    if (n_euc) memcpy(hi.data() + 6 * (size_t)n_id, i4, sizeof(int32_t) * 3 * n_euc);
    double *dd = (double *)blk; int32_t *di = (int32_t *)(dd + nd);
    PRE3_HIP(hipMemcpy(dd, hd.data(), sizeof(double) * nd, hipMemcpyHostToDevice));
    PRE3_HIP(hipMemcpy(di, hi.data(), sizeof(int32_t) * ni, hipMemcpyHostToDevice));
    hipLaunchKernelGGL(k_hyp_support, dim3(1), dim3(256), 0, 0, dd, to_camd(cam), n_id, di, di + 3 * (size_t)n_id, di + 5 * (size_t)n_id, dd + n,
                       n_euc, di + 6 * (size_t)n_id, dd + n + 2 * (size_t)n_id, threshold, dd + n + 2 * (size_t)m, di + 6 * (size_t)n_id + 3 * (size_t)n_euc);
    PRE3_HIP(hipGetLastError());
    PRE3_HIP(hipMemcpy(out_host, di + 6 * (size_t)n_id + 3 * (size_t)n_euc, sizeof(int32_t) * (1 + m), hipMemcpyDeviceToHost));
    return PRE3_OK;
}

}
```

### 3pre_amd/csrc/pre3_internal.h

```cpp
#pragma once
#include <hip/hip_runtime.h>
#include <cstdint>
#include <cstdio>
#include <cstring>
#include <string>
#include <vector>

#include "../../include/pre3.h"

namespace pre3 {

void set_error(const char *fmt, ...);

#define PRE3_HIP(call)                                                                         \
    do {                                                                                       \
        hipError_t e_ = (call);                                                                \
        if (e_ != hipSuccess) {                                                                \
            pre3::set_error("%s failed: %s (%s:%d)", #call, hipGetErrorString(e_), __FILE__, __LINE__); \
            return PRE3_E_HIP;                                                                 \
        }                                                                                      \
    } while (0)

#define PRE3_CHECK(cond, status, ...)                                                          \
    do {                                                                                       \
        if (!(cond)) { pre3::set_error(__VA_ARGS__); return (status); }                        \
    } while (0)

#define PRE3_TRY(expr)                                                                         \
    do { int rc_ = (expr); if (rc_ != PRE3_OK) return rc_; } while (0)

static inline int round_up(int v, int m) { return (v + m - 1) / m * m; }
static inline int ceil_div(int a, int b) { return (a + b - 1) / b; }

constexpr int TILE = 128;
constexpr int NB = 64;
constexpr int ELLW = 16;
constexpr int MAXK = 4;

#ifdef __HIPCC__
__device__ __forceinline__ float ell_fma(float a, float b, float c) { return __builtin_fmaf(a, b, c); }
__device__ __forceinline__ double ell_fma(double a, double b, double c) { return __builtin_fma(a, b, c); }
#endif

struct LmBuffers {
    int32_t *type = nullptr, *off = nullptr;
    double *h = nullptr;
    int32_t *has_h = nullptr;
    double *Hc = nullptr, *Hl = nullptr;
    double *S = nullptr;
    int32_t *has_S = nullptr;
    double *z = nullptr;
    int32_t *ic = nullptr, *li = nullptr, *hi = nullptr;
};

constexpr int RMAX = 16;
struct RowsBlock {
    int32_t r, applied, pad_[2];
    int32_t col[RMAX * RMAX];
    double val[RMAX * RMAX];
    double nu[RMAX];
    double R[RMAX * RMAX];
    double q[4];
};
struct HeadingSrc { double z[3]; double RR[9]; int32_t sta, pad_; };
struct RowsHeading { int on, strict; double z[3]; double RR[9]; const HeadingSrc *src; };

struct KernelTiming {
    bool enabled = false;
    int every = 1, seen = 0;
    std::vector<hipEvent_t> ev;
    int used = 0;
    double flops = 0, bytes = 0;
    int fused = 0; double fact_flops = 0; bool pending = false;
};

}

struct StepRequest {
    bool leave_jn_to_predict = false;
    bool pend_keep = false;
    bool defer_select = false;
    bool ride_innovation = false;
    bool ride_rescue_projection = false;
    bool want_gate_ride = false; double rescue_chi2 = 0.0;
    bool tail_want = false; double tail_chi2 = 0.0;
    const int32_t *book_from = nullptr;
};
struct LaunchOutcome {
    bool innovation_rode = false;
    bool rescue_projected = false;
    bool proj_with_jnorm = false;
    bool rescue_gated = false;
    bool cholp_done = false;
    bool tail_launched = false;
    bool x_done = false;
    bool jn_q_valid = false;
    bool proj_in_cholp = false;
    int dd_done = 0;
    int split_rows = 0;
};
struct Carried {
    bool hi_pending = false;
    int last_n_hi = 0;
    bool jn_pending = false;
    int pend_rows = 0;
    bool hi_pend_launched = false;
    bool hi_fused = false;
    bool tail_done = false;
    bool select_pending = false; int sel_n_draw = 0, sel_k = 0, sel_early_exit = 0;
};

struct pre3_ctx {
    int device = 0, dtype = PRE3_F32;
    size_t esz = 4;
    hipStream_t stream = nullptr;
    int capN = 0, capn = 0, capm = 0, caph = 0;
    int N = 0, n = 0;
    int ld = 0;
    int ldw = 0;
    int rcap = 0;
    pre3_cam cam{};
    bool have_cam = false;
    double *x_kk = nullptr, *x_km1 = nullptr;
    void *P = nullptr;
    void *tiles = nullptr;
    int n_tiles = 0;
    void *tiles_flat = nullptr;
    unsigned int *tile_ctr = nullptr;
    int *tile_cnt = nullptr; int tiles_stride = 0;
    bool tile_ctr_clean = false;
    int num_cus = 256;
    void *Wp = nullptr;
    bool k9_b3 = false;
    void *Sp = nullptr;
    void *tiles128 = nullptr; int n_tiles128 = 0;
    unsigned int *chol_arrive = nullptr; unsigned int chol_target = 0;
    unsigned int ride_target[2] = { 0, 0 };
    void *comm = nullptr; bool comm_owned = false;
    StepRequest req; LaunchOutcome out; Carried carry;
    bool defer_hi = false;
    int p_which = -1;
    bool x_valid[2] = {false, false};
    pre3::LmBuffers lm;
    int m = 0;
    std::vector<int32_t> meas_host;
    int32_t *meas = nullptr;
    int32_t *row_col = nullptr;
    void *row_val = nullptr;
    double *row_nu = nullptr;
    void *HP = nullptr;
    void *G = nullptr;
    void *W = nullptr;
    void *Smat = nullptr;
    void *Rdense = nullptr;
    int32_t *sel_rows = nullptr;
    int32_t *hyp = nullptr;
    int32_t *support = nullptr;
    uint32_t *masks = nullptr;
    int mask_words_cap = 0;
    int scored_n_draw = 0, scored_k = 0;
    int32_t *stats = nullptr;
    int32_t *li_meas = nullptr, *hi_meas = nullptr;
    double *pred_params = nullptr;
    int32_t *pinned_stats = nullptr;
    int32_t *mail_host = nullptr, *mail_dev = nullptr;
    int32_t seq_select = 0, seq_collect = 0;
    bool g_valid = false;
    int li_from_host = -1, hi_from_host = -1;
    bool li_kernel = false, hi_kernel = false;
    void *inbox_dev = nullptr; unsigned char *inbox_host = nullptr; void *inbox_host_dev = nullptr;
    size_t inbox_bytes = 0, off_meas = 0, off_ic = 0, off_hyp = 0, off_z = 0, off_flags = 0, flags_bytes = 0;
    int32_t seq_inbox = 0;
    bool inbox_pending = false;
    void *P_alt = nullptr; double *x_alt = nullptr; int32_t *map_col = nullptr; void *map_val = nullptr; int32_t *map_desc = nullptr; int32_t *map_src0 = nullptr; double *map_conv = nullptr;
    double *map_feat = nullptr; int32_t *map_flags = nullptr;
    void *map_stage[2] = { nullptr, nullptr }; hipEvent_t map_stage_ev[2] = { nullptr, nullptr }; bool map_stage_used[2] = { false, false };
    int map_stage_next = 0; size_t map_stage_bytes = 0;
    std::vector<int32_t> lm_type_host;
    double *bank = nullptr, *bank_alt = nullptr; bool bank_set = false;
    double *scan_desc = nullptr, *scan_pos = nullptr; int scan_K2 = 0, scan_cap = 0;
    void *up_stage[2] = { nullptr, nullptr }; hipEvent_t up_stage_ev[2] = { nullptr, nullptr }; bool up_stage_used[2] = { false, false };
    int up_stage_next = 0; size_t up_stage_bytes = 0;
    int32_t stage_seq[4] = { 0, 0, 0, 0 };
    void *ic_result_host = nullptr, *ic_result_host_dev = nullptr; int32_t seq_ic = 0;
    int32_t *ic_pred = nullptr, *ic_counts = nullptr, *ic_arg = nullptr, *ic_pairs = nullptr, *ic_newk2 = nullptr; double *ic_best = nullptr, *ic_second = nullptr;
    int32_t *bank_src = nullptr;
    int ic_route = 0;
    bool ic_last_ranked = false;
    void *ic_rank = nullptr; bool bank_ok = false;
    size_t ic_pcap = 0;
    double *ic_pb = nullptr, *ic_ps = nullptr; int32_t *ic_pa = nullptr;
    hipEvent_t t0 = nullptr, t1 = nullptr;
    pre3::KernelTiming kt;
    bool measurements_set = false, projected = false, innovated = false;
    int32_t *need = nullptr; int need_tag = 0;
    unsigned int *cholp_flags = nullptr; void *cholp_tp = nullptr; unsigned int cholp_epoch = 0; bool chol_persist = true;
    bool cholp_counted = false;
    int32_t *dd_groups = nullptr; int dd_n_groups = 0; void *dd_tiles = nullptr; std::vector<int> dd_tile_off;
    bool k9_overlap = true;
    bool shard_round = false;
    float *jn_q = nullptr;
    bool hp_all_valid = false;
    void *tail_yp = nullptr; float *tail_hb = nullptr; int32_t *tail_hib = nullptr; float *tail_wt = nullptr;
    bool pend_opt = false;
    unsigned long long *hf_sx = nullptr;
    float *W_pend = nullptr; void *Wp_pend = nullptr; unsigned *hf_xy = nullptr;
    bool step_tail = false;
    double *lmr_dev = nullptr, *lmr_host = nullptr;
    void *mset_dev = nullptr, *mset_host = nullptr; size_t mset_bytes = 0;
    pre3::RowsBlock *rows_blk = nullptr; double *rows_hp = nullptr;
    int rows_form = 0;
    void *plane_buf = nullptr; size_t plane_bytes = 0; pre3::HeadingSrc *plane_src = nullptr;
    bool booked = false; int book_s = 0;
    int32_t *book = nullptr, *book_alt = nullptr, *book_vis = nullptr;
    void *pol_dev = nullptr; size_t pol_dev_bytes = 0;
    int32_t *pol_host = nullptr, *pol_host_dev = nullptr; size_t pol_host_bytes = 0;
};

namespace pre3 {

__device__ inline void d_normjac(const double *q, double *J)
{
    double r = q[0], x = q[1], y = q[2], z = q[3];
    double s = pow(r * r + x * x + y * y + z * z, -1.5);
    J[0] = s * (x * x + y * y + z * z); J[1] = s * (-r * x); J[2] = s * (-r * y); J[3] = s * (-r * z);
    J[4] = s * (-x * r); J[5] = s * (r * r + y * y + z * z); J[6] = s * (-x * y); J[7] = s * (-x * z);
    J[8] = s * (-y * r); J[9] = s * (-y * x); J[10] = s * (r * r + x * x + z * z); J[11] = s * (-y * z);
    J[12] = s * (-z * r); J[13] = s * (-z * x); J[14] = s * (-z * y); J[15] = s * (r * r + x * x + y * y);
}

enum class Entry { ordinary, step, reader };
struct EntryScope {
    pre3_ctx *c; Entry kind; int rc;
    explicit EntryScope(pre3_ctx *c, Entry kind = Entry::ordinary, bool pend_keep = false);
    ~EntryScope();
    EntryScope(const EntryScope &) = delete;
};
int flush_unless_kept(pre3_ctx *c);
void drop_carried(pre3_ctx *c);
int dmalloc_bytes(void **p, size_t bytes);
int wait_mail(pre3_ctx *c, int slot, int32_t seq);
int stats_words(pre3_ctx *c);
int fetch_stats(pre3_ctx *c);
int install_measurements(pre3_ctx *c, int m, const int32_t *meas_idx, const double *z , const int32_t *hyp, int n_hyp_ints,
                         bool flags_clear = false, bool pull = true, size_t *nbytes_out = nullptr);
int set_descriptors_impl(pre3_ctx *c, int first, int count, const double *desc);
int update_hi_impl(pre3_ctx *c);

int scratch_acquire(size_t bytes, void **p_out, int *slot_out);
void scratch_release(int slot, void *p);
void release_scratch();
int match_partial(int device, int cls, int ND, int K1, const void *L1, int K2, const void *L2, int k2_offset, double *best, double *second, int32_t *arg);
int knn_run(int device, int D, int N, const double *data, int M, const double *query, int k, double *ids, double *dist);
void *match_bench_create(int cls, int ND, int K1, const void *L1, int K2, const void *L2);
int match_bench_info(void *h, int32_t info[3]);
int match_bench_run(void *h, int reps, double *ms_per);
int match_bench_fetch(void *h, double *best, double *second, int32_t *arg);
void match_bench_destroy(void *h);
void *match_shard_create(int device, int cls, int ND, int K1, const void *L1, int K2, const void *L2, int k2_offset);
int match_shard_run(void *h, void **partial_dev, int *n_doubles);
int match_shard_merge(void *h, int G, const void *gathered_dev, double thresh, double *pairs_out, double *score_out, int *M_out);
void match_shard_destroy(void *h);
int match_shard_set_comm(void *h, void *comm);
int match_shard_match(void *h, double thresh, double *pairs_out, double *score_out, int *M_out);
int match_shard_test_stall(void *h, int release);

int comm_all_reduce_i32(void *comm, void *buf, size_t count, hipStream_t st);
int comm_all_gather_f64(void *comm, const void *src, void *dst, size_t count_per_rank, hipStream_t st);
int comm_timeout_ms(void *comm);
int comm_give_up(void *comm, const char *what);
int comm_poll_error(void *comm);
int comm_abort_ms(void *comm);
bool comm_broken(void *comm);
bool comm_abort_wait(void *comm, int ms);
int stream_drain_on(hipStream_t st, void *comm, const char *what);
int stream_drain(pre3_ctx *c, const char *what);
void comm_rank_world(void *comm, int *rank, int *world);
int comm_device(void *comm);

int launch_ic_search(pre3_ctx *c, double thresh, int strict);
bool ic_search_fused_applies(const pre3_ctx *c);
int launch_ic_search_fused(pre3_ctx *c, double thresh, int strict, int32_t seq, int slot, bool matched);
int launch_bank_gather(pre3_ctx *c, int N_new, const int32_t *src_host);
int ic_rank_set_scan(pre3_ctx *c, bool in_bounds);
int launch_pull(pre3_ctx *c, const void *pinned_host, void *dst_dev, size_t bytes, int done_slot = -1);
int stage_wait(pre3_ctx *c, int k);
void ic_rank_free(pre3_ctx *c);
constexpr int DESC_DIM = 128;

int launch_project(pre3_ctx *c, int which, int clear_first);
int launch_innovation(pre3_ctx *c, int mode , double chi2, bool clear_flags = false, bool collect = true );
struct IcMatchRide;
int launch_project_innovation(pre3_ctx *c, int which, int clear_first, int mode, double chi2, bool collect = true, bool clear_ic = false, const IcMatchRide *ride = nullptr);
int launch_update_x(pre3_ctx *c, int which_prior, int r);
int launch_jnorm(pre3_ctx *c, int which);
int launch_predict_impl(pre3_ctx *c, const double u[7], bool with_projection = false, size_t inbox_n16 = 0, int32_t inbox_seq = 0);
int launch_inbox_pull(pre3_ctx *c, const void *src_host_mapped, void *dst_dev, size_t n16, int32_t seq, int slot = 10, int32_t *clear = nullptr, int n_clear = 0);
int launch_slice_prepare(pre3_ctx *c, const void *src_host_mapped, size_t n16, int32_t seq, int n_zero, int k, int lo, int hi, int tag);
int launch_window_gate(pre3_ctx *c, int M, const int32_t *pred_idx_dev, const int32_t *k1_dev, const double *zc_dev, int strict, int32_t *accept_dev);
int launch_build_rows_impl(pre3_ctx *c, int nsel, const int32_t *sel_dev, int r_pad);
int launch_ransac_score_impl(pre3_ctx *c, int k, double threshold, int hyp_begin, int hyp_end, int ldg, int32_t *support_dev, uint32_t *mask_dev, int mask_words,
                             int select_n_draw = 0, int early_exit = 0);
int launch_ransac_select_impl(pre3_ctx *c, int n_draw, int k, int early_exit, int32_t *support_dev, const uint32_t *mask_dev, int mask_words, int err_idx = -1);

int read_landmarks(pre3_ctx *c, int which, int first, int count, double *xyz, double *cov_xyz, double *cov_native, double *linearity);
int read_marginal(pre3_ctx *c, int which, int k, const int32_t *idx, const double *jn, double *x_out, double *P_out);
void free_readers(pre3_ctx *c);

int launch_rows_update(pre3_ctx *c, const RowsBlock *rows, const RowsHeading *hd);
int rows_applied(pre3_ctx *c, int32_t *applied_host);
void free_rows(pre3_ctx *c);

void free_plane(pre3_ctx *c);
int stage_acquire(pre3_ctx *c, size_t bytes, void **host, void **dev, int *slot);
int stage_release(pre3_ctx *c, int slot);

int launch_draw_1p(unsigned long long seed, unsigned long long seq, int n_draw, int m, int k, int32_t *hyp_dev, hipStream_t st);
int launch_draw_vo(unsigned long long seed, unsigned long long seq, int n_hyp, int pnum, const double *m1_dev, const double *m2_dev, int ms, int32_t *draws_dev,
                   int32_t *capped_dev , hipStream_t st);
int launch_draw_plane(unsigned long long seed, unsigned long long seq, int n_draw, int npts, const double *pts_dev, int32_t *draws_dev, hipStream_t st);
int launch_cand_order(unsigned long long seed, unsigned long long seq, int K, int box_w, int box_h, const double *raw_dev, double *keys_dev, int32_t *order_dev,
                      double *cand_out_dev, hipStream_t st);

struct SrFrameView {
    int device, rows, cols, mode, has_conf;
    const double *x, *y, *z, *img, *conf, *maxima;
    hipStream_t stream;
};
int sr_frame_view(pre3_sr_frame *f, SrFrameView *v);
struct SrKeypointView { int K, ldf, ND, gate, n_kept; const double *frm, *des; };
int sr_frame_keypoint_view(pre3_sr_frame *f, SrKeypointView *v);
int sr_frame_pair_work(pre3_sr_frame *f, size_t dev_bytes, size_t pin_bytes, void **dev, void **pin, hipEvent_t *ev);

int launch_book_vis(pre3_ctx *c);
void free_policy(pre3_ctx *c);

int run_hypothesis_support(int n, const double *xi, const pre3_cam &cam, int n_id, const int32_t *i1, const int32_t *i2, const int32_t *i3,
                           const double *z_id, int n_euc, const int32_t *i4, const double *z_euc, double threshold, int32_t *out_host );

int run_update(pre3_ctx *c, int which_prior, int r, bool dense_R, void *Kt_out_dev , bool prebuilt = false, bool first_done = false,
               bool hp_built = false );
int launch_ell_HP_build_sel(pre3_ctx *c, int nsel, const int32_t *sel_dev , void *dst);
int launch_chol_first_spec(pre3_ctx *c, int nsel_max);
struct InboxRide;
int launch_ell_HP_build(pre3_ctx *c, void *dst, const int32_t *need = nullptr, int need_tag = 0 ,
                        const InboxRide *ib = nullptr );
int launch_ell_G_hyp(pre3_ctx *c, int k, int lo, int hi, int ldg);
// ... 14 lines not shown
```

### 3pre_amd/csrc/pre3_update.hip

```cpp
#include <algorithm>
#include <atomic>
#include <cstdlib>

#include "pre3_internal.h"
#include "pre3_geomdev.h"
#include "pre3_chain.h"
#include "pre3_chain_async.h"
#ifndef PRE3_CHAIN_ASYNC_F64
#define PRE3_CHAIN_ASYNC_F64 0
#endif
#ifndef PRE3_CHAIN_ASYNC
#define PRE3_CHAIN_ASYNC 1
#endif
#include "pre3_cholp.h"

namespace pre3 {

template <typename T>
__global__ __launch_bounds__(256) void k_ell_HP(int r, int r_pad, const int32_t *__restrict__ row_col, const T *__restrict__ row_val,
                                                const double *__restrict__ row_nu, const T *__restrict__ P, int ld, T *__restrict__ dst,
                                                int ldw, int with_nu)
{
    int a = blockIdx.y;
    int j = blockIdx.x * blockDim.x + threadIdx.x;
    if (j >= ldw || a >= r_pad) return;
    T out = (T)0;
    if (a < r) {
        if (j < ld) {
            T s = (T)0;
#pragma unroll
            for (int t = 0; t < ELLW; ++t) {
                T v = row_val[a * ELLW + t];
                int c = row_col[a * ELLW + t];
                s += v * P[(size_t)c * ld + j];
            }
            out = s;
        } else if (j == ld && with_nu) {
            out = (T)row_nu[a];
        }
    }
    dst[(size_t)a * ldw + j] = out;
}

template <typename T>
__global__ __launch_bounds__(256) void k_ell_HP_build(int m, int r_pad, const int32_t *__restrict__ meas, const int32_t *__restrict__ lm_type,
                                                      const int32_t *__restrict__ lm_off, const double *__restrict__ Hc,
                                                      const double *__restrict__ Hl, const double *__restrict__ z, const double *__restrict__ h,
                                                      int32_t *__restrict__ row_col, T *__restrict__ row_val, double *__restrict__ row_nu,
                                                      const T *__restrict__ P, int ld, T *__restrict__ dst, int ldw, const int32_t *__restrict__ need, int need_tag,
                                                      int ny_build, InnovRide ir, const int32_t *__restrict__ sel = nullptr, InboxRide ib = InboxRide{})
{
    if (ib.n16 > 0 && blockIdx.y == gridDim.y - 1) { if (blockIdx.x == 0) inbox_pull_block(ib); return; }
    if ((int)blockIdx.y >= ny_build) { innov_ride_block<T>(ir, ((int)blockIdx.y - ny_build) * gridDim.x + blockIdx.x); return; }
    if (need != nullptr && (int)blockIdx.y < m && need[blockIdx.y] != need_tag) return;
    typedef T v4_t __attribute__((ext_vector_type(4)));
    const int sIdx = blockIdx.y;
    const int j = (blockIdx.x * blockDim.x + threadIdx.x) * 4;
    if (2 * sIdx >= r_pad) return;
    v4_t out0 = { (T)0, (T)0, (T)0, (T)0 }, out1 = out0;
    if (sIdx < m) {
        const int i = meas[sel ? sel[sIdx] : sIdx];
        const int d = lm_type[i] == PRE3_INVDEPTH ? 6 : 3, off = lm_off[i];
        T v0[13], v1[13]; int cc[13];
#pragma unroll
        for (int t = 0; t < 7; ++t) { cc[t] = t; v0[t] = (T)Hc[14 * i + t]; v1[t] = (T)Hc[14 * i + 7 + t]; }
#pragma unroll
        for (int t = 0; t < 6; ++t) { cc[7 + t] = t < d ? off + t : 0; v0[7 + t] = t < d ? (T)Hl[12 * i + t] : (T)0; v1[7 + t] = t < d ? (T)Hl[12 * i + 6 + t] : (T)0; }
        const double nu0 = z[2 * i] - h[2 * i], nu1 = z[2 * i + 1] - h[2 * i + 1];
        if (blockIdx.x == 0) {
            if (threadIdx.x < 2 * ELLW) {
                const int t = threadIdx.x & (ELLW - 1), c = threadIdx.x >> 4;
                int cv = 0; T vt = (T)0;
#pragma unroll
                for (int u = 0; u < 13; ++u) if (u == t) { cv = cc[u]; vt = c ? v1[u] : v0[u]; }
                row_col[(2 * sIdx + c) * ELLW + t] = cv; row_val[(2 * sIdx + c) * ELLW + t] = vt;
            }
            if (threadIdx.x == 0) { row_nu[2 * sIdx] = nu0; row_nu[2 * sIdx + 1] = nu1; }
        }
        if (j < ld) {
            v4_t pv[13];
#pragma unroll
            for (int t = 0; t < 13; ++t) pv[t] = *reinterpret_cast<const v4_t *>(P + (size_t)cc[t] * ld + j);
#pragma unroll
            for (int t = 0; t < 13; ++t) { out0 += v0[t] * pv[t]; out1 += v1[t] * pv[t]; }
        } else if (j == ld) {
            out0[0] = (T)nu0; out1[0] = (T)nu1;
        }
    } else if (blockIdx.x == 0) {
        if (threadIdx.x < 2 * ELLW) { row_col[2 * sIdx * ELLW + threadIdx.x] = 0; row_val[2 * sIdx * ELLW + threadIdx.x] = (T)0; }
        if (threadIdx.x == 0) { row_nu[2 * sIdx] = 0; row_nu[2 * sIdx + 1] = 0; }
    }
    if (j < ldw) {
        *reinterpret_cast<v4_t *>(dst + (size_t)(2 * sIdx) * ldw + j) = out0;
        *reinterpret_cast<v4_t *>(dst + (size_t)(2 * sIdx + 1) * ldw + j) = out1;
    }
}

#ifndef PRE3_PEND_KB
#define PRE3_PEND_KB 8
#endif
template <typename T, int MB, bool PEND = false>
__global__ __launch_bounds__(256) void k_ell_HP_build_mb(int m, int r_pad, const int32_t *__restrict__ meas, const int32_t *__restrict__ lm_type,
                                                         const int32_t *__restrict__ lm_off, const double *__restrict__ Hc,
                                                         const double *__restrict__ Hl, const double *__restrict__ z, const double *__restrict__ h,
                                                         int32_t *__restrict__ row_col, T *__restrict__ row_val, double *__restrict__ row_nu,
                                                         const T *__restrict__ P, int ld, T *__restrict__ dst, int ldw, const int32_t *__restrict__ need, int need_tag,
                                                         int ny_build, InnovRide ir, const int32_t *__restrict__ sel = nullptr, InboxRide ib = InboxRide{}, PendW pw = PendW{})
{
    if (ib.n16 > 0 && blockIdx.y == gridDim.y - 1) { if (blockIdx.x == 0) inbox_pull_block(ib); return; }
    if ((int)blockIdx.y >= ny_build) { innov_ride_block<T>(ir, ((int)blockIdx.y - ny_build) * gridDim.x + blockIdx.x); return; }
    typedef T v4_t __attribute__((ext_vector_type(4)));
    constexpr int PEND_MAX = 2 * NB;
    __shared__ __attribute__((aligned(16))) float gp[PEND ? MB * 2 * PEND_MAX : 1];
    __shared__ T cv[MB][2][16];
    __shared__ int ccs[MB][16];
    __shared__ int state[MB];
    __shared__ double nus[MB][2];
    const int s0 = blockIdx.y * MB, tid = threadIdx.x;
    if (tid < MB * 16) {
        const int mi = tid >> 4, t = tid & 15, sIdx = s0 + mi;
        int st = 0, cvv = 0; T a0 = (T)0, a1 = (T)0;
        if (2 * sIdx < r_pad && !(need != nullptr && sIdx < m && need[sIdx] != need_tag)) {
            st = 1;
            if (sIdx < m) {
                st = 2;
                const int i = meas[sel ? sel[sIdx] : sIdx];
                const int d = lm_type[i] == PRE3_INVDEPTH ? 6 : 3, off = lm_off[i];
                if (t < 7) { cvv = t; a0 = (T)Hc[14 * i + t]; a1 = (T)Hc[14 * i + 7 + t]; }
                else if (t < 13) { const int u = t - 7; cvv = u < d ? off + u : 0; a0 = u < d ? (T)Hl[12 * i + u] : (T)0; a1 = u < d ? (T)Hl[12 * i + 6 + u] : (T)0; }
                if (t == 13) { nus[mi][0] = z[2 * i] - h[2 * i]; nus[mi][1] = z[2 * i + 1] - h[2 * i + 1]; }
            } else if (t == 13) { nus[mi][0] = 0; nus[mi][1] = 0; }
        }
        cv[mi][0][t] = a0; cv[mi][1][t] = a1; ccs[mi][t] = cvv;
        if (t == 0) state[mi] = st;
    }
    __syncthreads();
    if (blockIdx.x == 0 && tid < MB * 2 * ELLW) {
        const int mi = tid / (2 * ELLW), c = (tid / ELLW) & 1, t = tid & (ELLW - 1), sIdx = s0 + mi;
        if (state[mi] != 0) {
            row_col[(2 * sIdx + c) * ELLW + t] = t < 13 ? ccs[mi][t] : 0;
            row_val[(2 * sIdx + c) * ELLW + t] = t < 13 ? cv[mi][c][t] : (T)0;
            if (t == 0) row_nu[2 * sIdx + c] = nus[mi][c];
        }
    }
    const int j = (blockIdx.x * blockDim.x + tid) * 4;
    const int prow = PEND ? (pw.rows < PEND_MAX ? pw.rows : PEND_MAX) : 0;
    int any = 0;
#pragma unroll
    for (int mi = 0; mi < MB; ++mi) any |= state[mi] == 2;
    constexpr int GB = PEND ? 2 : (MB < 4 ? MB : 4);
    v4_t pp[7], lp[GB][6];
    const bool inside = j < ld;
    auto load_lp = [&](const int h) {
#pragma unroll
        for (int u = 0; u < GB; ++u)
            if (state[h + u] == 2) {
#pragma unroll
                for (int t = 0; t < 6; ++t) lp[u][t] = *reinterpret_cast<const v4_t *>(P + (size_t)ccs[h + u][7 + t] * ld + j);
            }
    };
    if (inside && any) {
#pragma unroll
        for (int t = 0; t < 7; ++t) pp[t] = *reinterpret_cast<const v4_t *>(P + (size_t)t * ld + j);
        load_lp(0);
    }
    constexpr int KB = PRE3_PEND_KB;
    const bool corr = PEND && prow > 0 && (int)(blockIdx.x * blockDim.x * 4) < ld;
    const bool corr_t = corr && inside && any;
    v4_t wa[KB], wb[KB];
    auto loadw = [&](v4_t (&w)[KB], const int k0) {
#pragma unroll
        for (int u = 0; u < KB; ++u) { const int k = k0 + u < prow ? k0 + u : prow - 1; w[u] = *reinterpret_cast<const v4_t *>(reinterpret_cast<const T *>(pw.W) + (size_t)k * pw.ldw + j); }
    };
    v4_t out[MB][2];
    auto applyw = [&](const v4_t (&w)[KB], const int k0) {
#pragma unroll
        for (int u = 0; u < KB; ++u) {
            if (k0 + u < prow) {
#pragma unroll
                for (int mi = 0; mi < MB; ++mi) { out[mi][0] -= (T)gp[(k0 + u) * (2 * MB) + 2 * mi] * w[u]; out[mi][1] -= (T)gp[(k0 + u) * (2 * MB) + 2 * mi + 1] * w[u]; }
            }
        }
    };
    if (corr) {
        for (int e = tid; e < MB * prow; e += 256) {
            const int mi = e % MB, k = e / MB;
            float g0 = 0.f, g1 = 0.f;
            if (state[mi] == 2) {
                const float *wr = pw.W + (size_t)k * pw.ldw;
#pragma unroll
                for (int t = 0; t < 13; ++t) { const float wv = wr[ccs[mi][t]]; g0 += (float)cv[mi][0][t] * wv; g1 += (float)cv[mi][1][t] * wv; }
            }
            gp[k * (2 * MB) + 2 * mi] = g0; gp[k * (2 * MB) + 2 * mi + 1] = g1;
        }
        __syncthreads();
    }
    if (j >= ldw) return;
#pragma unroll
    for (int h = 0; h < MB; h += GB) {
        if (h > 0 && inside && any) load_lp(h);
#pragma unroll
        for (int u = 0; u < GB; ++u) {
            const int mi = h + u;
            v4_t out0 = { (T)0, (T)0, (T)0, (T)0 }, out1 = out0;
            if (state[mi] == 2) {
                if (inside) {
#pragma unroll
                    for (int t = 0; t < 7; ++t) { out0 += cv[mi][0][t] * pp[t]; out1 += cv[mi][1][t] * pp[t]; }
#pragma unroll
                    for (int t = 0; t < 6; ++t) { out0 += cv[mi][0][7 + t] * lp[u][t]; out1 += cv[mi][1][7 + t] * lp[u][t]; }
                } else if (j == ld) {
                    out0[0] = (T)nus[mi][0]; out1[0] = (T)nus[mi][1];
                }
            }
            out[mi][0] = out0; out[mi][1] = out1;
        }
    }
    if (corr_t) {
        asm volatile("" ::: "memory");
        loadw(wa, 0);
        for (int k0 = 0; k0 < prow; k0 += 2 * KB) {
            if (k0 + KB < prow) loadw(wb, k0 + KB);
            applyw(wa, k0);
            if (k0 + 2 * KB < prow) loadw(wa, k0 + 2 * KB);
            if (k0 + KB < prow) applyw(wb, k0 + KB);
        }
    }
#pragma unroll
    for (int mi = 0; mi < MB; ++mi) {
        const int sIdx = s0 + mi;
        if (state[mi] == 0) continue;
        *reinterpret_cast<v4_t *>(dst + (size_t)(2 * sIdx) * ldw + j) = out[mi][0];
        *reinterpret_cast<v4_t *>(dst + (size_t)(2 * sIdx + 1) * ldw + j) = out[mi][1];
    }
}

template <typename T>
__global__ __launch_bounds__(64) void k_ell_G(int r, int r_pad, const int32_t *__restrict__ row_col, const T *__restrict__ row_val,
                                              const T *__restrict__ HP, int ldw, T *__restrict__ dst, int ldg, int add_identity,
                                              const T *__restrict__ Rd, int lower_only)
{
    int a = blockIdx.y;
    int b = blockIdx.x * blockDim.x + threadIdx.x;
    if (b >= r_pad || a >= r_pad) return;
    T out;
    if (lower_only && (int)(blockIdx.x * blockDim.x) > a) {
        out = (T)0;
    } else if (a < r && b < r) {
        T s = (T)0;
#pragma unroll
        for (int t = 0; t < ELLW; ++t) s = ell_fma(row_val[b * ELLW + t], HP[(size_t)a * ldw + row_col[b * ELLW + t]], s);
        if (Rd) s += Rd[(size_t)a * r + b];
        else if (add_identity && a == b) s += (T)1;
        out = s;
    } else {
        out = (a == b) ? (T)1 : (T)0;
    }
    dst[(size_t)a * ldg + b] = out;
}

template <typename T>
__global__ __launch_bounds__(256) void k_ell_G_hyp(const int32_t *__restrict__ hyp, int k, int lo, int hi, const int32_t *__restrict__ row_col,
                                                   const T *__restrict__ row_val, const T *__restrict__ HP, int ldw, T *__restrict__ dst, int ldg)
{
    const int np = k * (2 * k + 1);
    const int g = blockIdx.x * blockDim.x + threadIdx.x;
    if (g >= (hi - lo) * np) return;
    const int h = lo + g / np, p = g - (g / np) * np;
    int i = 0;
    while ((i + 1) * (i + 2) / 2 <= p) ++i;
    const int j = p - i * (i + 1) / 2;
    const int ri = 2 * hyp[h * k + (i >> 1)] + (i & 1), rj = 2 * hyp[h * k + (j >> 1)] + (j & 1);
    const int a = ri > rj ? ri : rj, b = ri > rj ? rj : ri;
    T s = (T)0;
#pragma unroll
    for (int t = 0; t < ELLW; ++t) s = ell_fma(row_val[b * ELLW + t], HP[(size_t)a * ldw + row_col[b * ELLW + t]], s);
    dst[(size_t)a * ldg + b] = s;
}


template <typename T, typename XT>
__device__ __forceinline__ void chol_store_w_strip(const XT &X, T *__restrict__ W, int ldw, int J, int c0, void *__restrict__ Wp, int nst_total, int ld)
{
// ... 1607 lines not shown
#pragma unroll
    for (int i = 0; i < NB; ++i)
#pragma unroll
        for (int j = 0; j < NB; ++j)
#pragma unroll
            for (int e = 0; e < 16; ++e)
                pv[i][j][e] = P[(size_t)(R0 + i * 32 + (e & 3) + 8 * (e >> 2) + lrow) * ld + C0 + j * 32 + lcol];
    B3_MFMAS(A, B);
    B3_MFMAS(A2, B2);
#undef B3_STAGE
#undef B3_MFMAS
#undef B3_MMA
#undef B3_READ_FRAGS
    __syncthreads();
#ifdef PRE3_PROBE
    if (threadIdx.x == 0 && blockIdx.x < 2048) g_k9rt[blockIdx.x * 4 + 2] = __builtin_amdgcn_s_memrealtime();
    if (threadIdx.x == 0 && blockIdx.x == 7) { g_probe[1] = __builtin_amdgcn_s_memtime(); g_probe[3] = __builtin_amdgcn_s_memrealtime(); }
#endif
    typedef float f4_t __attribute__((ext_vector_type(4)));
    float (*patch)[36] = reinterpret_cast<float (*)[36]>(reinterpret_cast<float *>(smem) + wave * (2 * 32 * 36));
    float (*patchT)[36] = patch + 32;
    static_assert(B3_NBUF * 2 * B3_GRAN * 16 >= 4 * 2 * 32 * 36 * 4, "patches must fit in the ring");
#pragma unroll
    for (int i = 0; i < NB; ++i)
#pragma unroll
        for (int j = 0; j < NB; ++j) {
            const int gi = NB * wi + i, gj = NB * wj + j;
            if (diag && gi > gj) continue;
            const bool dblk = diag && gi == gj;
            const int r0 = R0 + i * 32, c0 = C0 + j * 32;
            if (dblk) {
#pragma unroll
                for (int e = 0; e < 16; ++e) {
                    const int lr = (e & 3) + 8 * (e >> 2) + lrow;
                    const float v = pv[i][j][e] - acc[i][j][e];
                    if (lr <= lcol) store_wt(P + (size_t)(r0 + lr) * ld + c0 + lcol, v, wt);
                    patch[lr][lcol] = v;
                }
                __builtin_amdgcn_s_waitcnt(0xc07f);
                __builtin_amdgcn_wave_barrier();
                const int rr = lane & 31, half = lane >> 5;
#pragma unroll
                for (int cc = 0; cc < 32; cc += 2) {
                    const int c = cc + half;
                    if (rr < c) store_wt(P + (size_t)(c0 + c) * ld + r0 + rr, patch[rr][c], wt);
                }
            } else {
#pragma unroll
                for (int g = 0; g < 4; ++g) {
                    f4_t v;
#pragma unroll
                    for (int t = 0; t < 4; ++t) { v[t] = pv[i][j][4 * g + t] - acc[i][j][4 * g + t]; patch[8 * g + lrow + t][lcol] = v[t]; }
                    *reinterpret_cast<f4_t *>(&patchT[lcol][8 * g + lrow]) = v;
                }
                __builtin_amdgcn_s_waitcnt(0xc07f);
                __builtin_amdgcn_wave_barrier();
                const int rr = lane >> 3, c4 = (lane & 7) * 4;
#pragma unroll
                for (int it = 0; it < 4; ++it) {
                    const int row = rr + 8 * it;
                    store_wt(reinterpret_cast<f4_t *>(P + (size_t)(r0 + row) * ld + c0 + c4), *reinterpret_cast<const f4_t *>(&patch[row][c4]), wt);
                    store_wt(reinterpret_cast<f4_t *>(P + (size_t)(c0 + row) * ld + r0 + c4), *reinterpret_cast<const f4_t *>(&patchT[row][c4]), wt);
                }
            }
            __builtin_amdgcn_s_waitcnt(0xc07f);
            __builtin_amdgcn_wave_barrier();
        }
}

__global__ __launch_bounds__(256) void k_downdate_b3(float *__restrict__ P, int ld, const bf16x8_t *__restrict__ Wp, int nst_total, int nst,
                                                      const float *__restrict__ W, int ldw, const int2 *__restrict__ tiles, XUpd xu, ProjRide pr)
{
    __shared__ __attribute__((aligned(16))) bf16x8_t smem[B3_NBUF * 2 * B3_GRAN];
    static_assert(sizeof(smem) >= 4 * 32 * 33 * sizeof(float) && sizeof(smem) >= sizeof(double) * (16 * 64 + 4), "patches and riders borrow the ring");
    if (xu.gate != nullptr) {
        if (xu.gate[8] != 1) return;
        nst = 2 * xu.gate[5] > NB ? 8 : 4;
    }
    if ((int)blockIdx.x >= xu.n_tiles) {
        __builtin_amdgcn_s_setprio(3);
        const int nx = xu.nx, rb = blockIdx.x - xu.n_tiles;
        if (rb < nx) {
            update_x_block<float>(rb, xu.n, xu.gate != nullptr ? 2 * xu.gate[5] : xu.r, W, ldw, ld, xu.x_prior, xu.x_out, xu.params, reinterpret_cast<double *>(smem));
            if (pr.n_blocks) ride_signal(pr.ctr);
        } else {
            proj_ride_block(pr, rb - nx);
        }
        return;
    }
    const int2 t = tiles[blockIdx.x];
#ifdef PRE3_PROBE
    if (threadIdx.x == 0 && blockIdx.x < 2048) {
        g_k9rt[blockIdx.x * 4] = __builtin_amdgcn_s_memrealtime();
        unsigned hw, xcc;
        asm volatile("s_getreg_b32 %0, hwreg(HW_REG_HW_ID)" : "=s"(hw));
        asm volatile("s_getreg_b32 %0, hwreg(HW_REG_XCC_ID)" : "=s"(xcc));
        g_k9hw[blockIdx.x] = (hw & 0xffff) | ((xcc & 0xf) << 16) | ((unsigned)(t.x >> 16) << 24);
    }
#endif
    if (t.x >> 16) b3_tile<128>(P, ld, Wp, nst_total, nst, t.x & 0xffff, t.y, smem, xu.wt != 0);
    else b3_tile<64>(P, ld, Wp, nst_total, nst, t.x, t.y, smem, xu.wt != 0);
#ifdef PRE3_PROBE
    if (threadIdx.x == 0 && blockIdx.x < 2048) g_k9rt[blockIdx.x * 4 + 3] = __builtin_amdgcn_s_memrealtime();
#endif
}

template <typename T>
__global__ void k_fill_w(T *W, size_t count, float scale)
{
    size_t i = (size_t)blockIdx.x * blockDim.x + threadIdx.x;
    if (i >= count) return;
    uint32_t h = (uint32_t)(i * 2654435761u) ^ 0x9e3779b9u;
    h ^= h >> 15; h *= 0x85ebca6bu; h ^= h >> 13;
    W[i] = (T)(((int)(h & 0xffff) - 32768) * (scale / 32768.0f));
}

#define DISPATCH_T(c, expr_f64, expr_f32) do { if ((c)->dtype == PRE3_F64) { expr_f64; } else { expr_f32; } } while (0)

int launch_ell_HP(pre3_ctx *c, int r, void *dst, bool with_nu)
{
    PRE3_TRY(pend_flush(c));
    int r_pad = round_up(r, NB);
    dim3 g(ceil_div(c->ldw, 256), r_pad), b(256);
    DISPATCH_T(c,
        hipLaunchKernelGGL(k_ell_HP<double>, g, b, 0, c->stream, r, r_pad, c->row_col, (const double *)c->row_val, c->row_nu,
                           (const double *)c->P, c->ld, (double *)dst, c->ldw, with_nu ? 1 : 0),
        hipLaunchKernelGGL(k_ell_HP<float>, g, b, 0, c->stream, r, r_pad, c->row_col, (const float *)c->row_val, c->row_nu,
                           (const float *)c->P, c->ld, (float *)dst, c->ldw, with_nu ? 1 : 0));
    PRE3_HIP(hipGetLastError());
    return PRE3_OK;
}

static inline int hp_build_mb() { static const int v = getenv("PRE3_HP_MB") ? atoi(getenv("PRE3_HP_MB")) : 1; return v; }

int launch_ell_HP_build_sel(pre3_ctx *c, int nsel, const int32_t *sel_dev, void *dst)
{
    PRE3_TRY(pend_flush(c));
    const int r_pad = round_up(2 * nsel, NB);
    if (r_pad == 0) return PRE3_OK;
    const int gx = ceil_div(c->ldw / 4, 256), ny = r_pad / 2;
    InnovRide ir{};
    if (c->req.ride_innovation && !c->out.innovation_rode && c->N > 0) {
        const int nb = ceil_div(c->N * 16, 256), rows = ceil_div(nb, gx);
        ir = InnovRide{ rows * gx, c->N, c->ld, (int)(c->flags_bytes / sizeof(int32_t)), c->lm.type, c->lm.off, c->lm.has_h, c->P, c->lm.Hc, c->lm.Hl,
                        c->lm.S, c->lm.has_S, (int32_t *)((unsigned char *)c->inbox_dev + c->off_flags) };
    }
    if (hp_build_mb() > 0) {
        constexpr int MBF = 4, MBD = 2;
        auto kd = k_ell_HP_build_mb<double, MBD>; auto kf = k_ell_HP_build_mb<float, MBF>;
        const int nyg = c->dtype == PRE3_F32 ? ceil_div(ny, MBF) : ceil_div(ny, MBD);
        dim3 g(gx, nyg + (ir.n_blocks ? ir.n_blocks / gx : 0)), b(256);
        DISPATCH_T(c,
            hipLaunchKernelGGL(kd, g, b, 0, c->stream, nsel, r_pad, c->meas, c->lm.type, c->lm.off, c->lm.Hc, c->lm.Hl, c->lm.z, c->lm.h,
                               c->row_col, (double *)c->row_val, c->row_nu, (const double *)c->P, c->ld, (double *)dst, c->ldw, (const int32_t *)nullptr, 0, nyg, ir, sel_dev, InboxRide{}, PendW{}),
            hipLaunchKernelGGL(kf, g, b, 0, c->stream, nsel, r_pad, c->meas, c->lm.type, c->lm.off, c->lm.Hc, c->lm.Hl, c->lm.z, c->lm.h,
                               c->row_col, (float *)c->row_val, c->row_nu, (const float *)c->P, c->ld, (float *)dst, c->ldw, (const int32_t *)nullptr, 0, nyg, ir, sel_dev, InboxRide{}, PendW{}));
        PRE3_HIP(hipGetLastError());
        if (ir.n_blocks) { c->out.innovation_rode = true; c->innovated = true; }
        return PRE3_OK;
    }
    dim3 g(gx, ny + (ir.n_blocks ? ir.n_blocks / gx : 0)), b(256);
    DISPATCH_T(c,
        hipLaunchKernelGGL(k_ell_HP_build<double>, g, b, 0, c->stream, nsel, r_pad, c->meas, c->lm.type, c->lm.off, c->lm.Hc, c->lm.Hl, c->lm.z, c->lm.h,
                           c->row_col, (double *)c->row_val, c->row_nu, (const double *)c->P, c->ld, (double *)dst, c->ldw, (const int32_t *)nullptr, 0, ny, ir, sel_dev),
        hipLaunchKernelGGL(k_ell_HP_build<float>, g, b, 0, c->stream, nsel, r_pad, c->meas, c->lm.type, c->lm.off, c->lm.Hc, c->lm.Hl, c->lm.z, c->lm.h,
                           c->row_col, (float *)c->row_val, c->row_nu, (const float *)c->P, c->ld, (float *)dst, c->ldw, (const int32_t *)nullptr, 0, ny, ir, sel_dev));
    PRE3_HIP(hipGetLastError());
    if (ir.n_blocks) { c->out.innovation_rode = true; c->innovated = true; }
    return PRE3_OK;
}

int launch_ell_HP_build(pre3_ctx *c, void *dst, const int32_t *need, int need_tag, const InboxRide *ib_in)
{
    const InboxRide ib = ib_in ? *ib_in : InboxRide{};
    const int ib_rows = ib.n16 > 0 ? 1 : 0;
    const int r_pad = round_up(2 * c->m, NB);
    const int gx = ceil_div(c->ldw / 4, 256), ny = r_pad / 2;
    InnovRide ir{};
    if (c->req.ride_innovation && !c->out.innovation_rode && c->N > 0) {
        const int nb = ceil_div(c->N * 16, 256), rows = ceil_div(nb, gx);
        ir = InnovRide{ rows * gx, c->N, c->ld, (int)(c->flags_bytes / sizeof(int32_t)), c->lm.type, c->lm.off, c->lm.has_h, c->P, c->lm.Hc, c->lm.Hl,
                        c->lm.S, c->lm.has_S, (int32_t *)((unsigned char *)c->inbox_dev + c->off_flags) };
    }
    PendW pw = pend_args(c);
    if (pw.rows > 0 && !(hp_build_mb() > 0 && c->dtype == PRE3_F32 && need == nullptr)) { PRE3_TRY(pend_flush(c)); pw = PendW{}; }
    if (pw.rows > 0) { ir.pend_W = pw.W; ir.pend_ldw = pw.ldw; ir.pend_rows = pw.rows; }
    if (hp_build_mb() > 0 && need == nullptr) {
        constexpr int MBF = 4, MBD = 2;
        static const int mbp = getenv("PRE3_PEND_MB") ? atoi(getenv("PRE3_PEND_MB")) : 4;
        const int mbf = pw.rows > 0 ? (mbp == 8 ? 8 : 4) : MBF;
        auto kd = k_ell_HP_build_mb<double, MBD>; auto kf = pw.rows > 0 ? (mbf == 8 ? k_ell_HP_build_mb<float, 8, true> : k_ell_HP_build_mb<float, 4, true>) : k_ell_HP_build_mb<float, MBF, false>;
        const int nyg = c->dtype == PRE3_F32 ? ceil_div(ny, mbf) : ceil_div(ny, MBD);
        dim3 g(gx, nyg + (ir.n_blocks ? ir.n_blocks / gx : 0) + ib_rows), b(256);
        DISPATCH_T(c,
            hipLaunchKernelGGL(kd, g, b, 0, c->stream, c->m, r_pad, c->meas, c->lm.type, c->lm.off, c->lm.Hc, c->lm.Hl, c->lm.z, c->lm.h,
                               c->row_col, (double *)c->row_val, c->row_nu, (const double *)c->P, c->ld, (double *)dst, c->ldw, need, need_tag, nyg, ir, (const int32_t *)nullptr, ib, PendW{}),
            hipLaunchKernelGGL(kf, g, b, 0, c->stream, c->m, r_pad, c->meas, c->lm.type, c->lm.off, c->lm.Hc, c->lm.Hl, c->lm.z, c->lm.h,
                               c->row_col, (float *)c->row_val, c->row_nu, (const float *)c->P, c->ld, (float *)dst, c->ldw, need, need_tag, nyg, ir, (const int32_t *)nullptr, ib, pw));
        PRE3_HIP(hipGetLastError());
        if (ir.n_blocks) { c->out.innovation_rode = true; c->innovated = true; }
        return PRE3_OK;
    }
    dim3 g(gx, ny + (ir.n_blocks ? ir.n_blocks / gx : 0) + ib_rows), b(256);
    DISPATCH_T(c,
        hipLaunchKernelGGL(k_ell_HP_build<double>, g, b, 0, c->stream, c->m, r_pad, c->meas, c->lm.type, c->lm.off, c->lm.Hc, c->lm.Hl, c->lm.z, c->lm.h,
                           c->row_col, (double *)c->row_val, c->row_nu, (const double *)c->P, c->ld, (double *)dst, c->ldw, need, need_tag, ny, ir, (const int32_t *)nullptr, ib),
        hipLaunchKernelGGL(k_ell_HP_build<float>, g, b, 0, c->stream, c->m, r_pad, c->meas, c->lm.type, c->lm.off, c->lm.Hc, c->lm.Hl, c->lm.z, c->lm.h,
                           c->row_col, (float *)c->row_val, c->row_nu, (const float *)c->P, c->ld, (float *)dst, c->ldw, need, need_tag, ny, ir, (const int32_t *)nullptr, ib));
    PRE3_HIP(hipGetLastError());
    if (ir.n_blocks) { c->out.innovation_rode = true; c->innovated = true; }
    return PRE3_OK;
}

int launch_ell_G(pre3_ctx *c, int r, const void *HPsrc, void *dst, int ldg, int add_identity, const void *Rdense, bool lower_only)
{
    int r_pad = round_up(r, NB);
    dim3 g(ceil_div(r_pad, 64), r_pad), b(64);
    DISPATCH_T(c,
        hipLaunchKernelGGL(k_ell_G<double>, g, b, 0, c->stream, r, r_pad, c->row_col, (const double *)c->row_val, (const double *)HPsrc,
                           c->ldw, (double *)dst, ldg, add_identity, (const double *)Rdense, lower_only ? 1 : 0),
        hipLaunchKernelGGL(k_ell_G<float>, g, b, 0, c->stream, r, r_pad, c->row_col, (const float *)c->row_val, (const float *)HPsrc,
                           c->ldw, (float *)dst, ldg, add_identity, (const float *)Rdense, lower_only ? 1 : 0));
    PRE3_HIP(hipGetLastError());
    return PRE3_OK;
}

int launch_ell_G_hyp(pre3_ctx *c, int k, int lo, int hi, int ldg)
{
    if (hi <= lo) return PRE3_OK;
    dim3 g(ceil_div((hi - lo) * k * (2 * k + 1), 256)), b(256);
    DISPATCH_T(c,
        hipLaunchKernelGGL(k_ell_G_hyp<double>, g, b, 0, c->stream, c->hyp, k, lo, hi, c->row_col, (const double *)c->row_val, (const double *)c->HP, c->ldw, (double *)c->G, ldg),
        hipLaunchKernelGGL(k_ell_G_hyp<float>, g, b, 0, c->stream, c->hyp, k, lo, hi, c->row_col, (const float *)c->row_val, (const float *)c->HP, c->ldw, (float *)c->G, ldg));
    PRE3_HIP(hipGetLastError());
    return PRE3_OK;
}

static int launch_chol_solve(pre3_ctx *c, int r_pad, bool first_done = false, bool predicted_prior = false, int r = -1 , int which_prior = -1)
{
    int nrb = r_pad / NB, nW = c->ldw / NB;
    c->out.split_rows = 0;
    if (first_done && c->out.cholp_done) {
        c->out.cholp_done = false;
        c->out.split_rows = nrb * NB;
        if (c->kt.pending) cholp_timing_rows(c, r > 0 ? r : r_pad);
        return PRE3_OK;
    }
    c->out.cholp_done = false; c->out.dd_done = 0; c->out.x_done = false;
    if (!first_done && (nrb >= 2 || predicted_prior) && cholp_usable(c, nrb)) return launch_cholp(c, nrb, nrb, r, which_prior);
    {
        const bool split = c->k9_b3 && c->dtype == PRE3_F32 && c->Wp != nullptr;
        static const int pro_env = getenv("PRE3_CHOL_PRO_B3") ? atoi(getenv("PRE3_CHOL_PRO_B3")) : 1;
        const bool pro_planes = split && pro_env && c->Sp != nullptr;
        static const int early_env = getenv("PRE3_CHOL_EARLY") ? atoi(getenv("PRE3_CHOL_EARLY")) : 1;
        const int rows_last = (early_env && r > 0 && r <= r_pad && r > r_pad - NB) ? r - (r_pad - NB) : 0;
        static const int trail_split = getenv("PRE3_CHOL_TRAIL_SPLIT") ? atoi(getenv("PRE3_CHOL_TRAIL_SPLIT")) : 4;
        auto n_trail = [&](int J) { const int nK = J >= 1 ? nrb - J - 1 : 0; return nK * (nK + 1) / 2 + nK * nW; };
        auto own_trail_at = [&](int J) { return pro_planes && trail_split > 0 && n_trail(J) > trail_split * 2 * c->num_cus; };
        static const int trail_p = std::min(4, std::max(1, getenv("PRE3_CHOL_TRAIL_P") ? atoi(getenv("PRE3_CHOL_TRAIL_P")) : 4));
        int Jt = 0;
        if (trail_p > 1 && own_trail_at(1)) { Jt = trail_p; while (Jt < nrb && own_trail_at(Jt)) Jt += trail_p; }
        for (int J = first_done ? 1 : 0; J < nrb; ++J) {
            const int nS = nrb - J - 1, nP = 1 + nS + nW;
            const bool paired = J >= 1 && J <= Jt;
            const int npend = !paired ? 1 : (J % trail_p == 0 ? trail_p : J % trail_p);
            const int nT = paired ? 0 : n_trail(J);
            const int ncb = (split && !pro_planes && J >= 1) ? c->ld / B3_T : 0;
            const bool own_trail = !paired && own_trail_at(J);
            if (own_trail)
                hipLaunchKernelGGL(k_chol_trail_b3, dim3(nT), dim3(256), 0, c->stream, (float *)c->Smat, r_pad, (float *)c->W, c->ldw, J - 1, J + 1, nrb, nW,
                                   c->Wp, c->rcap / B3_BK, c->Sp, c->rcap / NB, -1);
            const int nT_in = own_trail ? 0 : nT;
            dim3 g(nP + nT_in + 4 * ncb), bP(CH_NTH);
            c->chol_target += (unsigned)(nP - 1);
            const bool early = rows_last > 0 && rows_last <= NB - 8 && J == nrb - 1;
            if (early) {
                DISPATCH_T(c,
                    hipLaunchKernelGGL((k_chol_step<double, true>), g, bP, 0, c->stream, (double *)c->Smat, r_pad, (double *)c->W, c->ldw, J, nrb, nW, nP, c->stats + 6, c->chol_arrive, c->chol_target,
                                       nP + nT_in, nullptr, 0, 0, 0, nullptr, 0, nullptr, 0, rows_last, 1),
                    hipLaunchKernelGGL((k_chol_step<float, true>), g, bP, 0, c->stream, (float *)c->Smat, r_pad, (float *)c->W, c->ldw, J, nrb, nW, nP, c->stats + 6, c->chol_arrive, c->chol_target,
                                       nP + nT_in, split ? c->Wp : nullptr, c->rcap / B3_BK, ncb, c->ld, pro_planes ? c->Sp : nullptr, c->rcap / NB, nullptr, 0, rows_last, npend));
            } else {
            DISPATCH_T(c,
                hipLaunchKernelGGL(k_chol_step<double>, g, bP, 0, c->stream, (double *)c->Smat, r_pad, (double *)c->W, c->ldw, J, nrb, nW, nP, c->stats + 6, c->chol_arrive, c->chol_target,
                                   nP + nT_in, nullptr, 0, 0, 0, nullptr, 0, nullptr, 0, 0, 1),
                hipLaunchKernelGGL(k_chol_step<float>, g, bP, 0, c->stream, (float *)c->Smat, r_pad, (float *)c->W, c->ldw, J, nrb, nW, nP, c->stats + 6, c->chol_arrive, c->chol_target,
                                   nP + nT_in, split ? c->Wp : nullptr, c->rcap / B3_BK, ncb, c->ld, pro_planes ? c->Sp : nullptr, c->rcap / NB, nullptr, 0, 0, npend));
            }
            if (paired && J % trail_p == trail_p - 1 && J + 2 <= nrb - 1) {
                const int nK2 = nrb - (J + 2), nT2 = nK2 * (nK2 + 1) / 2 + nK2 * nW;
                static const int t128 = getenv("PRE3_CHOL_TRAIL_T128") ? atoi(getenv("PRE3_CHOL_TRAIL_T128")) : 2;
                if (t128 == 2) {
                    static std::atomic<bool> attr{ false };
                    if (!attr.exchange(true)) (void)hipFuncSetAttribute(reinterpret_cast<const void *>(k_chol_trail_b3l), hipFuncAttributeMaxDynamicSharedMemorySize, TL_NSLOT * TL_STAGE * 16);
                    hipLaunchKernelGGL(k_chol_trail_b3l, dim3(nK2 * (nK2 + 1) / 2 + ((nK2 + 1) / 2) * ((nW + 1) / 2)), dim3(256), TL_NSLOT * TL_STAGE * 16, c->stream, (float *)c->Smat, r_pad,
                                       (float *)c->W, c->ldw, J - trail_p + 1, J + 2, nrb, nW, c->Wp, c->rcap / B3_BK, c->Sp, c->rcap / NB, J);
                } else if (t128)
                    hipLaunchKernelGGL(k_chol_trail_b3w, dim3(nK2 * (nK2 + 1) / 2 + ((nK2 + 1) / 2) * ((nW + 1) / 2)), dim3(256), 0, c->stream, (float *)c->Smat, r_pad, (float *)c->W,
                                       c->ldw, J - trail_p + 1, J + 2, nrb, nW, c->Wp, c->rcap / B3_BK, c->Sp, c->rcap / NB, J);
                else
                hipLaunchKernelGGL(k_chol_trail_b3, dim3(nT2), dim3(256), 0, c->stream, (float *)c->Smat, r_pad, (float *)c->W, c->ldw, J - trail_p + 1, J + 2, nrb, nW,
                                   c->Wp, c->rcap / B3_BK, c->Sp, c->rcap / NB, J);
            }
        }
        if (split) c->out.split_rows = nrb * NB;
        PRE3_HIP(hipGetLastError());
        return PRE3_OK;
    }
}

static bool rescue_ride_open(const pre3_ctx *c) { return c->req.ride_rescue_projection && !c->out.rescue_projected && !c->out.proj_with_jnorm && c->N > 0; }

int launch_downdate(pre3_ctx *c, int r, const void *W, int which_prior, int planes_rows)
{
    int r_pad = round_up(r, NB);
    static const int wgs_per_cu = getenv("PRE3_K9_WGS") ? atoi(getenv("PRE3_K9_WGS")) : 3;
    const int gsz = std::min(c->n_tiles, wgs_per_cu * c->num_cus);
    dim3 g(gsz), b(256);
    static const int force = getenv("PRE3_K9_FORM") ? atoi(getenv("PRE3_K9_FORM")) : 0;
    const bool one_tile = force == 1 || (force == 0 && c->n_tiles <= 5 * c->num_cus);
    const bool use_b3 = c->k9_b3 && c->dtype == PRE3_F32 && c->Wp != nullptr;
    if (!use_b3 && !one_tile && which_prior >= 0) PRE3_TRY(launch_update_x(c, which_prior, r));
    if (!use_b3 && !one_tile) {
        if (!c->tile_ctr_clean) PRE3_HIP(hipMemsetAsync(c->tile_ctr, 0, sizeof(unsigned int) * 8, c->stream));
        c->tile_ctr_clean = false;
    }
    hipEvent_t e0 = nullptr, e1 = nullptr;
    const bool timed = c->kt.enabled && c->out.dd_done == 0 && r_pad >= 2 * NB && which_prior != PRE3_X_K_K && (c->kt.seen++ % c->kt.every) == 0;
    if (timed) {
        if ((size_t)c->kt.used + 2 > c->kt.ev.size()) {
            for (int i = 0; i < 2; ++i) { hipEvent_t e; PRE3_HIP(hipEventCreate(&e)); c->kt.ev.push_back(e); }
        }
        e0 = c->kt.ev[c->kt.used]; e1 = c->kt.ev[c->kt.used + 1];
        c->kt.used += 2;
        PRE3_HIP(hipEventRecord(e0, c->stream));
    }
    if (use_b3) {
        const int nst = std::min(r_pad / B3_BK, std::max(4, 2 * ceil_div(r, 2 * B3_BK))), nst_total = c->rcap / B3_BK;
        const int st0 = std::max(c->out.split_rows, planes_rows) / B3_BK;
        c->out.split_rows = 0;
        if (st0 < nst) {
            dim3 gs(c->ld / B3_T, nst - st0);
            hipLaunchKernelGGL(k_split_w, gs, b, 0, c->stream, (const float *)W, c->ldw, (bf16x8_t *)c->Wp, nst_total, st0);
        }
        const int2 *tiles = (const int2 *)c->tiles128;
        int n_tiles_launch = c->n_tiles128;
        if (c->out.dd_done > 0) {
            const int t0 = c->dd_tile_off[c->out.dd_done];
            tiles = (const int2 *)c->dd_tiles + t0;
            n_tiles_launch = c->dd_tile_off.back() - t0;
        }
        c->out.dd_done = 0;
        XUpd xu{ n_tiles_launch, c->n, r, which_prior == PRE3_X_K_K ? c->x_kk : c->x_km1, c->x_kk, c->pred_params, nullptr, 0 };
        xu.wt = k9_write_through();
        const bool x_done = c->out.x_done && which_prior >= 0;
        c->out.x_done = false;
        const int nx = (which_prior >= 0 && !x_done) ? ceil_div(c->n, 64) : 0;
        xu.nx = nx;
        ProjRide pr{};
        if (which_prior >= 0 && rescue_ride_open(c)) {
            if (n_tiles_launch + nx == 0) {
// ... 261 lines not shown
```

Baseline: 7348.

## Speed up RANSAC scoring: prepacked per-measurement records, lane-parallel solve, ballot masks

The HP-build kernel now also writes a packed per-measurement record (offset, type, z, state slice), which the RANSAC score kernel reads in one load instead of chasing meas/lm_type/lm_off/x/z. The small dense solve in the solver wave is spread across lanes: each lane holds one column and pivots via readlane broadcasts, replacing the single-lane serial elimination. The env var PRE3_RANSAC_SOLVE can switch back to the old path. For each thread's first measurement, the inlier mask is built with a wave ballot instead of shared-memory atomics. Timestamp probes are compiled in only under PRE3_PROBE. The cost is an extra buffer and extra writes in HP build.

```diff
diff --git a/3pre_amd/csrc/pre3_api.hip b/3pre_amd/csrc/pre3_api.hip
--- a/3pre_amd/csrc/pre3_api.hip
+++ b/3pre_amd/csrc/pre3_api.hip
@@ -318,6 +318,7 @@
     A(dmalloc_bytes(&c->G, (size_t)c->rcap * c->rcap * c->esz));
     A(dmalloc_bytes(&c->Smat, (size_t)c->rcap * c->rcap * c->esz));
     A(dmalloc(&c->sel_rows, c->rcap)); A(dmalloc(&c->need, c->capm));
+    { void *f = nullptr; A(dmalloc_bytes(&f, sizeof(ScoreRec) * (size_t)c->capm)); c->score_rec = (ScoreRec *)f; }
     if (rc == PRE3_OK) (void)hipMemset(c->need, 0, sizeof(int32_t) * c->capm);
     A(dmalloc(&c->support, (size_t)c->caph + 4 + (size_t)c->caph * c->mask_words_cap));
     if (rc == PRE3_OK) c->masks = reinterpret_cast<uint32_t *>(c->support + c->caph + 4);
@@ -457,7 +458,7 @@
     c->comm = nullptr;
     void *bufs[] = { c->x_kk, c->x_km1, c->P, c->lm.type, c->lm.off, c->lm.h, c->lm.has_h, c->lm.Hc, c->lm.Hl, c->lm.S, c->lm.has_S,
                      c->inbox_dev, c->row_col, c->row_val, c->row_nu, c->HP, c->W, c->G, c->Smat, c->Rdense,
-                     c->sel_rows, c->support, c->stats, c->pred_params, c->tiles, c->tile_ctr, c->tile_cnt, c->tiles_flat, c->P_alt, c->x_alt, c->map_col, c->map_val, c->map_desc, c->map_src0, c->map_conv, c->map_feat, c->map_flags, c->bank, c->bank_alt, c->scan_desc, c->scan_pos, c->ic_pred, c->ic_counts, c->ic_arg, c->ic_newk2, c->ic_best, c->ic_second, c->bank_src, c->chol_arrive, c->ic_pb, c->ic_ps, c->ic_pa, c->Wp, c->Sp, c->tiles128, c->need, c->cholp_flags, c->cholp_tp, c->dd_groups, c->dd_tiles, c->tail_yp, c->tail_hb, c->tail_hib, c->tail_wt, c->jn_q, c->W_pend, c->Wp_pend, c->hf_xy, c->hf_sx };
+                     c->sel_rows, c->support, c->stats, c->pred_params, c->tiles, c->tile_ctr, c->tile_cnt, c->tiles_flat, c->P_alt, c->x_alt, c->map_col, c->map_val, c->map_desc, c->map_src0, c->map_conv, c->map_feat, c->map_flags, c->bank, c->bank_alt, c->scan_desc, c->scan_pos, c->ic_pred, c->ic_counts, c->ic_arg, c->ic_newk2, c->ic_best, c->ic_second, c->bank_src, c->chol_arrive, c->ic_pb, c->ic_ps, c->ic_pa, c->Wp, c->Sp, c->tiles128, c->need, c->score_rec, c->cholp_flags, c->cholp_tp, c->dd_groups, c->dd_tiles, c->tail_yp, c->tail_hb, c->tail_hib, c->tail_wt, c->jn_q, c->W_pend, c->Wp_pend, c->hf_xy, c->hf_sx };
     for (void *b : bufs) if (b) (void)hipFree(b);
     free_readers(c);
     free_rows(c);
diff --git a/3pre_amd/csrc/pre3_geom.hip b/3pre_amd/csrc/pre3_geom.hip
--- a/3pre_amd/csrc/pre3_geom.hip
+++ b/3pre_amd/csrc/pre3_geom.hip
@@ -362,7 +362,19 @@
                                             int32_t *__restrict__ sel_rows, int32_t *__restrict__ stats,
                                             int32_t *mail, int seq, int err_idx = -1);
 
-template <typename T, int K>
+#ifdef PRE3_PROBE
+static __device__ unsigned long long g_sc[16];
+#define SC_STAMP(k, t) do { if (threadIdx.x == (t) && blockIdx.x == 5) g_sc[k] = __builtin_amdgcn_s_memrealtime(); } while (0)
+#else
+#define SC_STAMP(k, t)
+#endif
+
+__device__ __forceinline__ double lane_bcast(double v, int l)
+{
+    return __hiloint2double(__builtin_amdgcn_readlane(__double2hiint(v), l), __builtin_amdgcn_readlane(__double2loint(v), l));
+}
+
+template <typename T, int K, bool LANES>
 __global__ __launch_bounds__(512) void k_ransac_score(int hyp_begin, const int32_t *__restrict__ hyp, int m,
                                                       const int32_t *__restrict__ meas, const int32_t *__restrict__ lm_type,
                                                       const int32_t *__restrict__ lm_off, const double *__restrict__ x,
@@ -370,7 +382,8 @@
                                                       const double *__restrict__ row_nu, const double *__restrict__ z,
                                                       CamD cam, double threshold, int32_t *support,
                                                       uint32_t *masks, int mask_words, SelArgs sel,
-                                                      const int32_t *__restrict__ row_col, const T *__restrict__ row_val)
+                                                      const int32_t *__restrict__ row_col, const T *__restrict__ row_val,
+                                                      const ScoreRec *__restrict__ rec )
 {
     constexpr int R = 2 * K;
     extern __shared__ double s_res[];
@@ -400,13 +413,24 @@
     int i0 = 0, type0 = PRE3_INVDEPTH;
     T hpl[R][6];
     double xl[6], z0 = 0, z1 = 0;
+    SC_STAMP(0, 448);
     if (have0) {
-        i0 = meas[tid];
-        type0 = lm_type[i0];
-        const int off = lm_off[i0];
+        int off;
+        struct __attribute__((packed, aligned(8))) X6 { double v[6]; };
+        X6 xv;
+        if (rec != nullptr) {
+            const ScoreRec r = rec[tid];
+            off = r.off; type0 = r.type; z0 = r.z[0]; z1 = r.z[1];
+#pragma unroll
+            for (int c = 0; c < 6; ++c) xv.v[c] = r.x[c];
+        } else {
+            i0 = meas[tid];
+            type0 = lm_type[i0];
+            off = lm_off[i0];
+            xv = *reinterpret_cast<const X6 *>(x + off);
+            z0 = z[2 * i0]; z1 = z[2 * i0 + 1];
+        }
         struct __attribute__((packed, aligned(sizeof(T)))) Row6 { T v[6]; };
-        struct __attribute__((packed, aligned(8))) X6 { double v[6]; };
-        const X6 xv = *reinterpret_cast<const X6 *>(x + off);
 #pragma unroll
         for (int b = 0; b < R; ++b) {
             const Row6 rv = *reinterpret_cast<const Row6 *>(hp[b] + off);
@@ -415,11 +439,9 @@
         }
 #pragma unroll
         for (int c = 0; c < 6; ++c) xl[c] = (c < 3 || type0 == PRE3_INVDEPTH) ? xv.v[c] : 0.0;
-        z0 = z[2 * i0]; z1 = z[2 * i0 + 1];
     }
     const int solver = (int)(blockDim.x >> 6) - 1;
     if (wv == solver) {
-        double A[R][R + 1];
         T gv = (T)0;
         if (G == nullptr) {
             int pi = 0;
@@ -440,53 +462,112 @@
                 for (int t = 0; t < ELLW; ++t) gv = ell_fma(vv[t], hv[t], gv);
             }
         }
-#pragma unroll
-        for (int a = 0; a < R; ++a) {
-#pragma unroll
-            for (int b = 0; b < R; ++b) {
+#ifdef PRE3_PROBE
+        asm volatile("s_waitcnt vmcnt(0)" ::: "memory");
+#endif
+        SC_STAMP(1, 448);
+        if constexpr (LANES) {
+            const int bb = lane < R ? lane : R;
+            int rowb = rows[0];
+#pragma unroll
+            for (int a = 1; a < R; ++a) if (a == bb) rowb = rows[a];
+            double col[R];
+#pragma unroll
+            for (int a = 0; a < R; ++a) {
+                double v;
                 if (G != nullptr) {
-                    const int ra = rows[a] > rows[b] ? rows[a] : rows[b], rb = rows[a] > rows[b] ? rows[b] : rows[a];
-                    A[a][b] = (double)G[(size_t)ra * ldg + rb] + (a == b ? 1.0 : 0.0);
+                    const int ra = rows[a] > rowb ? rows[a] : rowb, rb = rows[a] > rowb ? rowb : rows[a];
+                    v = (double)G[(size_t)ra * ldg + rb] + (a == bb ? 1.0 : 0.0);
                 } else {
-                    const int hi_ = a > b ? a : b, lo_ = a > b ? b : a;
-                    A[a][b] = (double)__shfl(gv, hi_ * (hi_ + 1) / 2 + lo_, 64) + (a == b ? 1.0 : 0.0);
+                    const int hi_ = a > bb ? a : bb, lo_ = a > bb ? bb : a;
+                    v = (double)__shfl(gv, hi_ * (hi_ + 1) / 2 + lo_, 64) + (a == bb ? 1.0 : 0.0);
                 }
-            }
-            A[a][R] = row_nu[rows[a]];
-        }
-        if (lane == 0) {
+                const double nu = row_nu[rows[a]];
+                col[a] = bb == R ? nu : v;
+            }
 #pragma unroll
             for (int c = 0; c < R; ++c) {
-                int p = c; double best = fabs(A[c][c]);
-#pragma unroll
-                for (int a = c + 1; a < R; ++a) { double v = fabs(A[a][c]); if (v > best) { best = v; p = a; } }
+                double pc[R];
+#pragma unroll
+                for (int a = c; a < R; ++a) pc[a] = lane_bcast(col[a], c);
+                int p = c; double best = fabs(pc[c]);
+#pragma unroll
+                for (int a = c + 1; a < R; ++a) { double v = fabs(pc[a]); if (v > best) { best = v; p = a; } }
 #pragma unroll
                 for (int a = c + 1; a < R; ++a)
-                    if (a == p) {
-#pragma unroll
-                        for (int b = 0; b <= R; ++b) { double t = A[c][b]; A[c][b] = A[a][b]; A[a][b] = t; }
+                    if (a == p) { double t = col[c]; col[c] = col[a]; col[a] = t; t = pc[c]; pc[c] = pc[a]; pc[a] = t; }
+                const double dinv = 1.0 / pc[c];
+#pragma unroll
+                for (int a = c + 1; a < R; ++a) {
+                    const double l = pc[a] * dinv;
+                    col[a] -= l * col[c];
+                }
+            }
+            double w[R];
+#pragma unroll
+            for (int a = R - 1; a >= 0; --a) {
+                double s = lane_bcast(col[a], R);
+#pragma unroll
+                for (int b = a + 1; b < R; ++b) s -= lane_bcast(col[a], b) * w[b];
+                w[a] = s / lane_bcast(col[a], a);
+            }
+            if (lane == 0) {
+#pragma unroll
+                for (int a = 0; a < R; ++a) s_w[a] = w[a];
+            }
+        } else {
+            double A[R][R + 1];
+#pragma unroll
+            for (int a = 0; a < R; ++a) {
+#pragma unroll
+                for (int b = 0; b < R; ++b) {
+                    if (G != nullptr) {
+                        const int ra = rows[a] > rows[b] ? rows[a] : rows[b], rb = rows[a] > rows[b] ? rows[b] : rows[a];
+                        A[a][b] = (double)G[(size_t)ra * ldg + rb] + (a == b ? 1.0 : 0.0);
+                    } else {
+                        const int hi_ = a > b ? a : b, lo_ = a > b ? b : a;
+                        A[a][b] = (double)__shfl(gv, hi_ * (hi_ + 1) / 2 + lo_, 64) + (a == b ? 1.0 : 0.0);
                     }
-                const double dinv = 1.0 / A[c][c];
-#pragma unroll
-                for (int a = c + 1; a < R; ++a) {
-                    const double l = A[a][c] * dinv;
-#pragma unroll
-                    for (int b = c + 1; b <= R; ++b) A[a][b] -= l * A[c][b];
                 }
-            }
-            double w[R];
-#pragma unroll
-            for (int a = R - 1; a >= 0; --a) {
-                double s = A[a][R];
-#pragma unroll
-                for (int b = a + 1; b < R; ++b) s -= A[a][b] * w[b];
-                w[a] = s / A[a][a];
-            }
-#pragma unroll
-            for (int a = 0; a < R; ++a) s_w[a] = w[a];
-        }
-    }
-    __syncthreads();
+                A[a][R] = row_nu[rows[a]];
+            }
+            if (lane == 0) {
+#pragma unroll
+                for (int c = 0; c < R; ++c) {
+                    int p = c; double best = fabs(A[c][c]);
+#pragma unroll
+                    for (int a = c + 1; a < R; ++a) { double v = fabs(A[a][c]); if (v > best) { best = v; p = a; } }
+#pragma unroll
+                    for (int a = c + 1; a < R; ++a)
+                        if (a == p) {
+#pragma unroll
+                            for (int b = 0; b <= R; ++b) { double t = A[c][b]; A[c][b] = A[a][b]; A[a][b] = t; }
+                        }
+                    const double dinv = 1.0 / A[c][c];
+#pragma unroll
+                    for (int a = c + 1; a < R; ++a) {
+                        const double l = A[a][c] * dinv;
+#pragma unroll
+                        for (int b = c + 1; b <= R; ++b) A[a][b] -= l * A[c][b];
+                    }
+                }
+                double w[R];
+#pragma unroll
+                for (int a = R - 1; a >= 0; --a) {
+                    double s = A[a][R];
+#pragma unroll
+                    for (int b = a + 1; b < R; ++b) s -= A[a][b] * w[b];
+                    w[a] = s / A[a][a];
+                }
+#pragma unroll
+                for (int a = 0; a < R; ++a) s_w[a] = w[a];
+            }
+        }
+        SC_STAMP(2, 448);
+    }
+    SC_STAMP(8, 0);
+    __syncthreads();
+    SC_STAMP(3, 0);
     double w[R];
 #pragma unroll
     for (int b = 0; b < R; ++b) w[b] = s_w[b];
@@ -501,6 +582,7 @@
     double rot[9];
     d_q2r(xc + 3, rot);
     double lmin = INFINITY;
+    int typeF = PRE3_INVDEPTH; double resF = 0;
     for (int j = tid; j < m; j += blockDim.x) {
         const bool pre = PRE_POSE && j == tid;
         const int i = pre ? i0 : meas[j];
@@ -524,28 +606,38 @@
         d_pinhole_distort(hc, cam, uvd);
         const double n0 = (pre ? z0 : z[2 * i]) - uvd[0], n1 = (pre ? z1 : z[2 * i + 1]) - uvd[1];
         const double res = sqrt(n0 * n0 + n1 * n1);
-        s_res[j] = res;
+        if (j == tid) { typeF = type; resF = res; } else s_res[j] = res;
         if (type == PRE3_INVDEPTH) lmin = fmin(lmin, res);
     }
+    SC_STAMP(4, 0);
     lmin = wave_min(lmin);
     if (lane == 0) s_red[wv] = lmin;
     uint32_t *s_mask = (uint32_t *)(s_res + m);
-    for (int wd = tid; wd < mask_words; wd += blockDim.x) s_mask[wd] = 0;
+    const bool tail = m > (int)blockDim.x;
+    if (tail) for (int wd = tid; wd < mask_words; wd += blockDim.x) s_mask[wd] = 0;
     __syncthreads();
     double minres = s_red[0];
     for (int w2 = 1; w2 < (int)(blockDim.x >> 6); ++w2) minres = fmin(minres, s_red[w2]);
+    SC_STAMP(5, 0);
+    const int in0 = tid < m && ((typeF == PRE3_INVDEPTH) ? (resF < (minres + threshold)) : (resF < threshold));
+    const unsigned long long bal = __ballot(in0);
+    if (lane == 0) {
+        if (2 * wv < mask_words) s_mask[2 * wv] = (uint32_t)bal;
+        if (2 * wv + 1 < mask_words) s_mask[2 * wv + 1] = (uint32_t)(bal >> 32);
+    }
     int cnt = 0;
-    for (int j = tid; j < m; j += blockDim.x) {
+    for (int j = tid + blockDim.x; j < m; j += blockDim.x) {
         const int type = lm_type[meas[j]];
         const double res = s_res[j];
         const int in = (type == PRE3_INVDEPTH) ? (res < (minres + threshold)) : (res < threshold);
         if (in) { atomicOr(&s_mask[j >> 5], 1u << (j & 31)); ++cnt; }
     }
-    cnt = wave_sum(cnt);
-    if (lane == 0) s_cnt[wv] = cnt;
+    if (tail) cnt = wave_sum(cnt);
+    if (lane == 0) s_cnt[wv] = cnt + __popcll(bal);
     __syncthreads();
     if (tid == 0) { int sc = 0; for (int w2 = 0; w2 < (int)(blockDim.x >> 6); ++w2) sc += s_cnt[w2]; support[hidx] = sc; }
     for (int wd = tid; wd < mask_words; wd += blockDim.x) masks[(size_t)hidx * mask_words + wd] = s_mask[wd];
+    SC_STAMP(6, 0);
     if (sel.fuse) {
         __shared__ int s_last;
         __syncthreads();
@@ -1071,13 +1163,18 @@
                            uint32_t *mask_dev, int mask_words, const SelArgs &sel)
 {
 #define SCORE_ARGS hyp_begin, c->hyp, c->m, c->meas, c->lm.type, c->lm.off, c->x_km1, (const T *)c->HP, c->ldw, c->g_valid ? (const T *)c->G : (const T *)nullptr, ldg, \
-                   c->row_nu, c->lm.z, to_camd(c->cam), threshold, support_dev, mask_dev, mask_words, sel, c->row_col, (const T *)c->row_val
+                   c->row_nu, c->lm.z, to_camd(c->cam), threshold, support_dev, mask_dev, mask_words, sel, c->row_col, (const T *)c->row_val, \
+                   c->score_rec_valid ? (const ScoreRec *)c->score_rec : (const ScoreRec *)nullptr
+    static const int lanes_env = getenv("PRE3_RANSAC_SOLVE") ? atoi(getenv("PRE3_RANSAC_SOLVE")) : 1;
+#define SCORE_CASE(KK) if (lanes_env) hipLaunchKernelGGL((k_ransac_score<T, KK, true>), dim3(nb), dim3(SCORE_THREADS), shm, c->stream, SCORE_ARGS); \
+                       else hipLaunchKernelGGL((k_ransac_score<T, KK, false>), dim3(nb), dim3(SCORE_THREADS), shm, c->stream, SCORE_ARGS)
     switch (k) {
-    case 1: hipLaunchKernelGGL((k_ransac_score<T, 1>), dim3(nb), dim3(SCORE_THREADS), shm, c->stream, SCORE_ARGS); break;
-    case 2: hipLaunchKernelGGL((k_ransac_score<T, 2>), dim3(nb), dim3(SCORE_THREADS), shm, c->stream, SCORE_ARGS); break;
-    case 3: hipLaunchKernelGGL((k_ransac_score<T, 3>), dim3(nb), dim3(SCORE_THREADS), shm, c->stream, SCORE_ARGS); break;
-    default: hipLaunchKernelGGL((k_ransac_score<T, 4>), dim3(nb), dim3(SCORE_THREADS), shm, c->stream, SCORE_ARGS); break;
-    }
+    case 1: SCORE_CASE(1); break;
+    case 2: SCORE_CASE(2); break;
+    case 3: SCORE_CASE(3); break;
+    default: SCORE_CASE(4); break;
+    }
+#undef SCORE_CASE
 #undef SCORE_ARGS
 }
 
@@ -1262,4 +1359,11 @@
     return PRE3_OK;
 }
 
-}
+#ifdef PRE3_PROBE
+extern "C" __attribute__((visibility("default"))) int pre3_debug_sc(unsigned long long *out)
+{
+    return hipMemcpyFromSymbol(out, HIP_SYMBOL(g_sc), sizeof(unsigned long long) * 16) == hipSuccess ? 0 : -3;
+}
+#endif
+
+}
diff --git a/3pre_amd/csrc/pre3_internal.h b/3pre_amd/csrc/pre3_internal.h
--- a/3pre_amd/csrc/pre3_internal.h
+++ b/3pre_amd/csrc/pre3_internal.h
@@ -41,6 +41,9 @@
 __device__ __forceinline__ float ell_fma(float a, float b, float c) { return __builtin_fmaf(a, b, c); }
 __device__ __forceinline__ double ell_fma(double a, double b, double c) { return __builtin_fma(a, b, c); }
 #endif
+
+struct alignas(16) ScoreRec { int32_t off, type; double z[2]; double x[6]; };
+struct ScoreRecOut { ScoreRec *rec; const double *x; };
 
 struct LmBuffers {
     int32_t *type = nullptr, *off = nullptr;
@@ -193,6 +196,7 @@
     hipEvent_t t0 = nullptr, t1 = nullptr;
     pre3::KernelTiming kt;
     bool measurements_set = false, projected = false, innovated = false;
+    pre3::ScoreRec *score_rec = nullptr; bool score_rec_valid = false;
     int32_t *need = nullptr; int need_tag = 0;
     unsigned int *cholp_flags = nullptr; void *cholp_tp = nullptr; unsigned int cholp_epoch = 0; bool chol_persist = true;
     bool cholp_counted = false;
diff --git a/3pre_amd/csrc/pre3_update.hip b/3pre_amd/csrc/pre3_update.hip
--- a/3pre_amd/csrc/pre3_update.hip
+++ b/3pre_amd/csrc/pre3_update.hip
@@ -48,7 +48,7 @@
                                                       const double *__restrict__ Hl, const double *__restrict__ z, const double *__restrict__ h,
                                                       int32_t *__restrict__ row_col, T *__restrict__ row_val, double *__restrict__ row_nu,
                                                       const T *__restrict__ P, int ld, T *__restrict__ dst, int ldw, const int32_t *__restrict__ need, int need_tag,
-                                                      int ny_build, InnovRide ir, const int32_t *__restrict__ sel = nullptr, InboxRide ib = InboxRide{})
+                                                      int ny_build, InnovRide ir, const int32_t *__restrict__ sel = nullptr, InboxRide ib = InboxRide{}, ScoreRecOut so = ScoreRecOut{})
 {
     if (ib.n16 > 0 && blockIdx.y == gridDim.y - 1) { if (blockIdx.x == 0) inbox_pull_block(ib); return; }
     if ((int)blockIdx.y >= ny_build) { innov_ride_block<T>(ir, ((int)blockIdx.y - ny_build) * gridDim.x + blockIdx.x); return; }
@@ -76,6 +76,12 @@
                 row_col[(2 * sIdx + c) * ELLW + t] = cv; row_val[(2 * sIdx + c) * ELLW + t] = vt;
             }
             if (threadIdx.x == 0) { row_nu[2 * sIdx] = nu0; row_nu[2 * sIdx + 1] = nu1; }
+            if (threadIdx.x == 2 * ELLW && so.rec != nullptr) {
+                ScoreRec rc; rc.off = off; rc.type = lm_type[i]; rc.z[0] = z[2 * i]; rc.z[1] = z[2 * i + 1];
+#pragma unroll
+                for (int t = 0; t < 6; ++t) rc.x[t] = t < d ? so.x[off + t] : 0.0;
+                so.rec[sIdx] = rc;
+            }
         }
         if (j < ld) {
             v4_t pv[13];
@@ -105,7 +111,7 @@
                                                          const double *__restrict__ Hl, const double *__restrict__ z, const double *__restrict__ h,
                                                          int32_t *__restrict__ row_col, T *__restrict__ row_val, double *__restrict__ row_nu,
                                                          const T *__restrict__ P, int ld, T *__restrict__ dst, int ldw, const int32_t *__restrict__ need, int need_tag,
-                                                         int ny_build, InnovRide ir, const int32_t *__restrict__ sel = nullptr, InboxRide ib = InboxRide{}, PendW pw = PendW{})
+                                                         int ny_build, InnovRide ir, const int32_t *__restrict__ sel = nullptr, InboxRide ib = InboxRide{}, PendW pw = PendW{}, ScoreRecOut so = ScoreRecOut{})
 {
     if (ib.n16 > 0 && blockIdx.y == gridDim.y - 1) { if (blockIdx.x == 0) inbox_pull_block(ib); return; }
     if ((int)blockIdx.y >= ny_build) { innov_ride_block<T>(ir, ((int)blockIdx.y - ny_build) * gridDim.x + blockIdx.x); return; }
@@ -129,6 +135,12 @@
                 if (t < 7) { cvv = t; a0 = (T)Hc[14 * i + t]; a1 = (T)Hc[14 * i + 7 + t]; }
                 else if (t < 13) { const int u = t - 7; cvv = u < d ? off + u : 0; a0 = u < d ? (T)Hl[12 * i + u] : (T)0; a1 = u < d ? (T)Hl[12 * i + 6 + u] : (T)0; }
                 if (t == 13) { nus[mi][0] = z[2 * i] - h[2 * i]; nus[mi][1] = z[2 * i + 1] - h[2 * i + 1]; }
+                if (t == 14 && blockIdx.x == 0 && so.rec != nullptr) {
+                    ScoreRec rc; rc.off = off; rc.type = lm_type[i]; rc.z[0] = z[2 * i]; rc.z[1] = z[2 * i + 1];
+#pragma unroll
+                    for (int u = 0; u < 6; ++u) rc.x[u] = u < d ? so.x[off + u] : 0.0;
+                    so.rec[sIdx] = rc;
+                }
             } else if (t == 13) { nus[mi][0] = 0; nus[mi][1] = 0; }
         }
         cv[mi][0][t] = a0; cv[mi][1][t] = a1; ccs[mi][t] = cvv;
@@ -2042,9 +2054,9 @@
         dim3 g(gx, nyg + (ir.n_blocks ? ir.n_blocks / gx : 0)), b(256);
         DISPATCH_T(c,
             hipLaunchKernelGGL(kd, g, b, 0, c->stream, nsel, r_pad, c->meas, c->lm.type, c->lm.off, c->lm.Hc, c->lm.Hl, c->lm.z, c->lm.h,
-                               c->row_col, (double *)c->row_val, c->row_nu, (const double *)c->P, c->ld, (double *)dst, c->ldw, (const int32_t *)nullptr, 0, nyg, ir, sel_dev, InboxRide{}, PendW{}),
+                               c->row_col, (double *)c->row_val, c->row_nu, (const double *)c->P, c->ld, (double *)dst, c->ldw, (const int32_t *)nullptr, 0, nyg, ir, sel_dev, InboxRide{}, PendW{}, ScoreRecOut{}),
             hipLaunchKernelGGL(kf, g, b, 0, c->stream, nsel, r_pad, c->meas, c->lm.type, c->lm.off, c->lm.Hc, c->lm.Hl, c->lm.z, c->lm.h,
-                               c->row_col, (float *)c->row_val, c->row_nu, (const float *)c->P, c->ld, (float *)dst, c->ldw, (const int32_t *)nullptr, 0, nyg, ir, sel_dev, InboxRide{}, PendW{}));
+                               c->row_col, (float *)c->row_val, c->row_nu, (const float *)c->P, c->ld, (float *)dst, c->ldw, (const int32_t *)nullptr, 0, nyg, ir, sel_dev, InboxRide{}, PendW{}, ScoreRecOut{}));
         PRE3_HIP(hipGetLastError());
         if (ir.n_blocks) { c->out.innovation_rode = true; c->innovated = true; }
         return PRE3_OK;
@@ -2064,6 +2076,8 @@
 {
     const InboxRide ib = ib_in ? *ib_in : InboxRide{};
     const int ib_rows = ib.n16 > 0 ? 1 : 0;
+    const ScoreRecOut so{ need == nullptr ? c->score_rec : nullptr, c->x_km1 };
+    c->score_rec_valid = so.rec != nullptr;
     const int r_pad = round_up(2 * c->m, NB);
     const int gx = ceil_div(c->ldw / 4, 256), ny = r_pad / 2;
     InnovRide ir{};
@@ -2084,9 +2098,9 @@
         dim3 g(gx, nyg + (ir.n_blocks ? ir.n_blocks / gx : 0) + ib_rows), b(256);
         DISPATCH_T(c,
             hipLaunchKernelGGL(kd, g, b, 0, c->stream, c->m, r_pad, c->meas, c->lm.type, c->lm.off, c->lm.Hc, c->lm.Hl, c->lm.z, c->lm.h,
-                               c->row_col, (double *)c->row_val, c->row_nu, (const double *)c->P, c->ld, (double *)dst, c->ldw, need, need_tag, nyg, ir, (const int32_t *)nullptr, ib, PendW{}),
+                               c->row_col, (double *)c->row_val, c->row_nu, (const double *)c->P, c->ld, (double *)dst, c->ldw, need, need_tag, nyg, ir, (const int32_t *)nullptr, ib, PendW{}, so),
             hipLaunchKernelGGL(kf, g, b, 0, c->stream, c->m, r_pad, c->meas, c->lm.type, c->lm.off, c->lm.Hc, c->lm.Hl, c->lm.z, c->lm.h,
-                               c->row_col, (float *)c->row_val, c->row_nu, (const float *)c->P, c->ld, (float *)dst, c->ldw, need, need_tag, nyg, ir, (const int32_t *)nullptr, ib, pw));
+                               c->row_col, (float *)c->row_val, c->row_nu, (const float *)c->P, c->ld, (float *)dst, c->ldw, need, need_tag, nyg, ir, (const int32_t *)nullptr, ib, pw, so));
         PRE3_HIP(hipGetLastError());
         if (ir.n_blocks) { c->out.innovation_rode = true; c->innovated = true; }
         return PRE3_OK;
@@ -2094,9 +2108,9 @@
     dim3 g(gx, ny + (ir.n_blocks ? ir.n_blocks / gx : 0) + ib_rows), b(256);
     DISPATCH_T(c,
         hipLaunchKernelGGL(k_ell_HP_build<double>, g, b, 0, c->stream, c->m, r_pad, c->meas, c->lm.type, c->lm.off, c->lm.Hc, c->lm.Hl, c->lm.z, c->lm.h,
-                           c->row_col, (double *)c->row_val, c->row_nu, (const double *)c->P, c->ld, (double *)dst, c->ldw, need, need_tag, ny, ir, (const int32_t *)nullptr, ib),
+                           c->row_col, (double *)c->row_val, c->row_nu, (const double *)c->P, c->ld, (double *)dst, c->ldw, need, need_tag, ny, ir, (const int32_t *)nullptr, ib, so),
         hipLaunchKernelGGL(k_ell_HP_build<float>, g, b, 0, c->stream, c->m, r_pad, c->meas, c->lm.type, c->lm.off, c->lm.Hc, c->lm.Hl, c->lm.z, c->lm.h,
-                           c->row_col, (float *)c->row_val, c->row_nu, (const float *)c->P, c->ld, (float *)dst, c->ldw, need, need_tag, ny, ir, (const int32_t *)nullptr, ib));
+                           c->row_col, (float *)c->row_val, c->row_nu, (const float *)c->P, c->ld, (float *)dst, c->ldw, need, need_tag, ny, ir, (const int32_t *)nullptr, ib, so));
     PRE3_HIP(hipGetLastError());
     if (ir.n_blocks) { c->out.innovation_rode = true; c->innovated = true; }
     return PRE3_OK;
```

New measurement: 7378 (median of 2 runs). About the same (+0.4%).
